# yezhen17/3DIoUMatch

Measured on AMD Instinct MI355X. Metric: scenes/sec train-step (ScanNet 40k pts, 256 proposals), higher is better.
Workload: dtype f32

## Files before the change

### 3dioumatch_amd/csrc/loss_core.h

```cpp
#pragma once
#include <math.h>

#ifndef LOSS_HD
#define LOSS_HD inline
#endif

#include "../../include/loss_hip.h"

typedef VnLossTensor LossTensor;
typedef VnLossArgs LossArgs;

LOSS_HD float lt_at(const LossTensor &t, int b, int k, int c, int d = 0) {
  return t.p[b * t.sb + k * t.sk + c * t.sc + d * t.sd];
}

enum {
  ACC_MASK, ACC_CE_MASK, ACC_POS, ACC_OBJACC, ACC_CENTER1, ACC_HCLS, ACC_HREG, ACC_SCLS, ACC_SREG,
  ACC_SEM, ACC_CLSACC, ACC_IOULAB, ACC_IOULAB_OBJ, ACC_IOUACC, ACC_IOUACC_OBJ, ACC_IOUHUB,
  ACC_JITACC, ACC_JITHUB, ACC_BLM, ACC_DIST2, ACC_VMASK, ACC_VDIST, ACC_COUNT
};

enum {
  ST_LOSS = VN_ST_LOSS, ST_VOTE = VN_ST_VOTE, ST_OBJ = VN_ST_OBJ, ST_CENTER = VN_ST_CENTER,
  ST_HCLS = VN_ST_HCLS, ST_HREG = VN_ST_HREG, ST_SCLS = VN_ST_SCLS, ST_SREG = VN_ST_SREG,
  ST_SEM = VN_ST_SEM, ST_BOX = VN_ST_BOX, ST_IOU = VN_ST_IOU, ST_JIT = VN_ST_JIT,
  ST_POS_RATIO = VN_ST_POS_RATIO, ST_NEG_RATIO = VN_ST_NEG_RATIO, ST_OBJ_ACC = VN_ST_OBJ_ACC,
  ST_OBJ_COUNT = VN_ST_OBJ_COUNT, ST_CLS_ACC = VN_ST_CLS_ACC, ST_PRED_IOU = VN_ST_PRED_IOU,
  ST_PRED_IOU_OBJ = VN_ST_PRED_IOU_OBJ, ST_IOU_ACC = VN_ST_IOU_ACC,
  ST_IOU_ACC_OBJ = VN_ST_IOU_ACC_OBJ, ST_JIT_ACC = VN_ST_JIT_ACC,
  ST_JIT_ACC_OBJ = VN_ST_JIT_ACC_OBJ, ST_COUNT = VN_ST_COUNT
};

constexpr int kLossBlock = 256;
LOSS_HD int loss_blocks_per_scene(int k, int s) {
  return (k + kLossBlock - 1) / kLossBlock + 1 + (s + kLossBlock - 1) / kLossBlock;
}

constexpr float kLossWeight = 10.0f;
constexpr float kNear = 0.3f, kFar = 0.6f;

LOSS_HD float huber1(float x) {
  const float a = fabsf(x);
  return a <= 1.0f ? 0.5f * x * x : a - 0.5f;
}
LOSS_HD float huber1_grad(float x) { return x > 1.0f ? 1.0f : (x < -1.0f ? -1.0f : x); }

constexpr int kRowMax = 32;

struct ScoreRow {
  float v[kRowMax];
};

LOSS_HD void load_row(const LossTensor &t, int b, int k, int n, ScoreRow &r) {
#pragma unroll
  for (int j = 0; j < kRowMax; ++j) r.v[j] = j < n ? lt_at(t, b, k, j) : -INFINITY;
}

LOSS_HD float row_log_sum_exp(const ScoreRow &r) {
  float m = r.v[0];
#pragma unroll
  for (int j = 1; j < kRowMax; ++j) m = r.v[j] > m ? r.v[j] : m;
  float s = 0.0f;
#pragma unroll
  for (int j = 0; j < kRowMax; ++j) s += expf(r.v[j] - m);
  return m + logf(s);
}

LOSS_HD float log_sum_exp(const LossTensor &t, int b, int k, int n) {
  float m = lt_at(t, b, k, 0);
  for (int j = 1; j < n; ++j) { const float v = lt_at(t, b, k, j); m = v > m ? v : m; }
  float s = 0.0f;
  for (int j = 0; j < n; ++j) s += expf(lt_at(t, b, k, j) - m);
  return m + logf(s);
}

LOSS_HD int arg_max(const LossTensor &t, int b, int k, int n) {
  int best = 0;
  float m = lt_at(t, b, k, 0);
  for (int j = 1; j < n; ++j) { const float v = lt_at(t, b, k, j); if (v > m) { m = v; best = j; } }
  return best;
}

LOSS_HD int row_arg_max(const LossTensor &t, int b, int k, int n) {
  if (n > kRowMax) return arg_max(t, b, k, n);
  ScoreRow r;
  load_row(t, b, k, n, r);
  int best = 0;
  float m = r.v[0];
#pragma unroll
  for (int j = 1; j < kRowMax; ++j)
    if (r.v[j] > m) { m = r.v[j]; best = j; }
  return best;
}

LOSS_HD float ce_and_grad(const LossTensor &t, int b, int k, int n, int label, float scale, float *g,
                          int *top) {
  if (n <= kRowMax) {
    ScoreRow r;
    load_row(t, b, k, n, r);
    const float lse = row_log_sum_exp(r);
    float at_label = 0.0f, m = r.v[0];
    int best = 0;
#pragma unroll
    for (int j = 0; j < kRowMax; ++j) {
      if (j < n) {
        g[j] = scale * (expf(r.v[j] - lse) - (j == label ? 1.0f : 0.0f));
        if (j == label) at_label = r.v[j];
        if (r.v[j] > m) { m = r.v[j]; best = j; }
      }
    }
    *top = best;
    return lse - at_label;
  }
  const float lse = log_sum_exp(t, b, k, n);
  for (int j = 0; j < n; ++j)
    g[j] = scale * (expf(lt_at(t, b, k, j) - lse) - (j == label ? 1.0f : 0.0f));
  *top = arg_max(t, b, k, n);
  return lse - lt_at(t, b, k, label);
}

LOSS_HD float class2angle(int cls, float residual, int nh) {
  if (nh == 1) return 0.0f;
  const float per = (float)(2.0 * M_PI / (double)nh);
  float angle = (float)cls * per + residual;
  if (angle > (float)M_PI) angle = angle - (float)(2.0 * M_PI);
  return angle;
}

LOSS_HD void decode_prediction(const LossArgs &a, int b, int k) {
  const int rows = a.has_jitter ? 2 * a.K : a.K;
  float *o = a.boxes + ((long long)b * rows + k) * 7;
  const int hc = row_arg_max(a.h_scores, b, k, a.NH);
  const int sc = row_arg_max(a.s_scores, b, k, a.NS);
  const float h_res = lt_at(a.h_resn, b, k, hc) * (float)(M_PI / (double)a.NH);
  for (int d = 0; d < 3; ++d) {
    o[d] = lt_at(a.center, b, k, d);
    const float mean = a.mean_size[sc * 3 + d];
    float s = mean + lt_at(a.s_resn, b, k, sc, d) * mean;
    if (s <= 0.0f) s = 1e-6f;
    o[3 + d] = s;
  }
  o[6] = -class2angle(hc, h_res, a.NH);
  if (a.has_jitter) {
    float *j = a.boxes + ((long long)b * rows + a.K + k) * 7;
    for (int d = 0; d < 3; ++d) {
      j[d] = lt_at(a.jit_center, b, k, d);
      j[3 + d] = lt_at(a.jit_size, b, k, d);
    }
    j[6] = -lt_at(a.jit_heading, b, k, 0);
  }
}

LOSS_HD void decode_ground_truth(const LossArgs &a, int b, int g) {
  const long long i = (long long)b * a.G + g;
  float *o = a.gt_boxes + i * 7;
  const bool empty = a.box_label_mask[i] != 1.0f;
  const int sc = (int)a.size_class_label[i];
  for (int d = 0; d < 3; ++d) {
    o[d] = empty ? -1000.0f : a.center_label[i * 3 + d];
    o[3 + d] = a.mean_size[sc * 3 + d] + a.size_residual_label[i * 3 + d];
  }
  o[6] = -class2angle((int)a.heading_class_label[i], a.heading_residual_label[i], a.NH);
}

struct SceneView {
  const float *gt_center;
  const float *gt_mask;
  const float *center;
  const int *nearest;
};

LOSS_HD void loss_proposal(const LossArgs &a, const SceneView &sv, int b, int k, float *acc) {
  const long long bk = (long long)b * a.K + k;
  const float vx = lt_at(a.agg_xyz, b, k, 0), vy = lt_at(a.agg_xyz, b, k, 1), vz = lt_at(a.agg_xyz, b, k, 2);
  const float cx = lt_at(a.center, b, k, 0), cy = lt_at(a.center, b, k, 1), cz = lt_at(a.center, b, k, 2);
  float best = 0.0f, best_c = 0.0f;
  int assign = 0, near_c = 0;
  for (int g = 0; g < a.G; ++g) {
    const float gx = sv.gt_center[g * 3], gy = sv.gt_center[g * 3 + 1], gz = sv.gt_center[g * 3 + 2];
    const bool empty = sv.gt_mask[g] != 1.0f;
    const float mx = empty ? -1000.0f : gx, my = empty ? -1000.0f : gy, mz = empty ? -1000.0f : gz;
    const float d = ((vx - mx) * (vx - mx) + (vy - my) * (vy - my)) + (vz - mz) * (vz - mz);
    if (g == 0 || d < best) { best = d; assign = g; }
    const float dc = ((cx - gx) * (cx - gx) + (cy - gy) * (cy - gy)) + (cz - gz) * (cz - gz);
    if (g == 0 || dc < best_c) { best_c = dc; near_c = g; }
  }
  const float dist = sqrtf(best + 1e-6f);
  const int label = dist < kNear ? 1 : 0;
  const float mask = (dist < kNear || dist > kFar) ? 1.0f : 0.0f;
  const float obj = (float)label;
  a.objectness_label[bk] = label;
  a.objectness_mask[bk] = mask;
  a.object_assignment[bk] = assign;
  acc[ACC_MASK] += mask;
  acc[ACC_POS] += obj;

  {
    const float w = label ? 0.8f : 0.2f;
    const float s0 = lt_at(a.obj, b, k, 0), s1 = lt_at(a.obj, b, k, 1);
    const float m = s0 > s1 ? s0 : s1;
    const float lse = m + logf(expf(s0 - m) + expf(s1 - m));
    const float scale = (a.consistency ? 0.0f : 0.5f * kLossWeight) * mask * w;
    a.g_obj[bk * 2] = scale * (expf(s0 - lse) - (label == 0 ? 1.0f : 0.0f));
    a.g_obj[bk * 2 + 1] = scale * (expf(s1 - lse) - (label == 1 ? 1.0f : 0.0f));
    acc[ACC_CE_MASK] += w * (lse - (label ? s1 : s0)) * mask;
    acc[ACC_OBJACC] += ((s1 > s0 ? 1 : 0) == label ? 1.0f : 0.0f) * mask;
  }
  {
    acc[ACC_CENTER1] += best_c * obj;
    const float s = kLossWeight * obj * 2.0f;
    a.g_center[bk * 3 + 0] = s * (cx - sv.gt_center[near_c * 3 + 0]);
    a.g_center[bk * 3 + 1] = s * (cy - sv.gt_center[near_c * 3 + 1]);
    a.g_center[bk * 3 + 2] = s * (cz - sv.gt_center[near_c * 3 + 2]);
  }
  const long long gi = (long long)b * a.G + assign;
  {
    const int hl = (int)a.heading_class_label[gi];
    float *gs = a.g_h_scores + bk * a.NH, *gr = a.g_h_resn + bk * a.NH;
    int top;
    acc[ACC_HCLS] += obj * ce_and_grad(a.h_scores, b, k, a.NH, hl, 0.1f * kLossWeight * obj, gs, &top);
    const float target = a.heading_residual_label[gi] / (float)(M_PI / (double)a.NH);
    const float x = lt_at(a.h_resn, b, k, hl) - target;
    acc[ACC_HREG] += obj * huber1(x);
    for (int j = 0; j < a.NH; ++j) gr[j] = j == hl ? kLossWeight * obj * huber1_grad(x) : 0.0f;
  }
  {
    const int sl = (int)a.size_class_label[gi];
    float *gs = a.g_s_scores + bk * a.NS, *gr = a.g_s_resn + bk * a.NS * 3;
    int top;
    acc[ACC_SCLS] += obj * ce_and_grad(a.s_scores, b, k, a.NS, sl, 0.1f * kLossWeight * obj, gs, &top);
    for (int j = 0; j < a.NS * 3; ++j) gr[j] = 0.0f;
    float reg = 0.0f;
    for (int d = 0; d < 3; ++d) {
      const float x = lt_at(a.s_resn, b, k, sl, d) - a.size_residual_label[gi * 3 + d] / a.mean_size[sl * 3 + d];
      reg += huber1(x);
      gr[sl * 3 + d] = kLossWeight * obj * huber1_grad(x) / 3.0f;
    }
    acc[ACC_SREG] += obj * (reg / 3.0f);
  }
  {
    const int cl = (int)a.sem_cls_label[gi];
    int top;
    acc[ACC_SEM] += obj * ce_and_grad(a.sem, b, k, a.NC, cl, 0.1f * kLossWeight * obj,
                                      a.g_sem + bk * a.NC, &top);
    acc[ACC_CLSACC] += obj * (top == cl ? 1.0f : 0.0f);
  }
  if (a.consistency) return;
  const int rows = a.has_jitter ? 2 * a.K : a.K;
  {
    const long long r = (long long)b * rows + k;
    const float lab = a.iou_lab[r];
    const int sel = a.NI > 1 ? (int)a.sem_cls_label[(long long)b * a.G + a.iou_assign[r]] : 0;
    const float p = 1.0f / (1.0f + expf(-lt_at(a.iou, b, k, sel)));
    const float x = p - lab;
    acc[ACC_IOULAB] += lab;
    acc[ACC_IOULAB_OBJ] += lab * obj;
    acc[ACC_IOUACC] += fabsf(x);
    acc[ACC_IOUACC_OBJ] += fabsf(x) * obj;
    acc[ACC_IOUHUB] += huber1(x);
    const float s = a.grad_scale * kLossWeight / (float)(a.B * a.K) * huber1_grad(x) * p * (1.0f - p);
    for (int j = 0; j < a.NI; ++j) a.g_iou[bk * a.NI + j] = j == sel ? s : 0.0f;
  }
  if (a.has_jitter) {
    const long long r = (long long)b * rows + a.K + k;
    const float lab = a.iou_lab[r];
    const int sel = a.NI > 1 ? (int)a.sem_cls_label[(long long)b * a.G + a.iou_assign[r]] : 0;
    const float p = 1.0f / (1.0f + expf(-lt_at(a.iou_jit, b, k, sel)));
    const float x = p - lab;
    acc[ACC_JITACC] += fabsf(x);
    acc[ACC_JITHUB] += huber1(x);
    const float s = a.grad_scale * kLossWeight / ((float)(a.B * a.K) + 1e-6f) * huber1_grad(x) * p * (1.0f - p);
    for (int j = 0; j < a.NI; ++j) a.g_iou_jit[bk * a.NI + j] = j == sel ? s : 0.0f;
  }
}

LOSS_HD void loss_ground_truth(const LossArgs &a, const SceneView &sv, int b, int g, float *acc) {
  const long long i = (long long)b * a.G + g;
  const float gx = sv.gt_center[g * 3], gy = sv.gt_center[g * 3 + 1], gz = sv.gt_center[g * 3 + 2];
  float best = 0.0f;
  int arg = 0;
  for (int k = 0; k < a.K; ++k) {
    const float cx = sv.center[k * 3], cy = sv.center[k * 3 + 1], cz = sv.center[k * 3 + 2];
    const float d = ((cx - gx) * (cx - gx) + (cy - gy) * (cy - gy)) + (cz - gz) * (cz - gz);
    if (k == 0 || d < best) { best = d; arg = k; }
  }
  a.gt_nearest[i] = arg;
  acc[ACC_BLM] += sv.gt_mask[g];
  acc[ACC_DIST2] += best * sv.gt_mask[g];
}

LOSS_HD int loss_seed(const LossArgs &a, int b, int s, float *acc, float *m) {
  const int p = a.seed_inds[b * a.seed_inds_stride + s];
  const long long row = (long long)b * a.N + p;
  const float mask = (float)a.vote_label_mask[row];
  float best = 0.0f;
  int arg = 0;
  for (int j = 0; j < a.VF; ++j)
    for (int g = 0; g < 3; ++g) {
      float d = 0.0f;
      for (int c = 0; c < 3; ++c)
        d += fabsf(lt_at(a.vote_xyz, b, s * a.VF + j, c) -
                   (a.vote_label[row * 9 + g * 3 + c] + lt_at(a.seed_xyz, b, s, c)));
      if ((j == 0 && g == 0) || d < best) { best = d; arg = j * 3 + g; }
    }
  acc[ACC_VMASK] += mask;
  acc[ACC_VDIST] += best * mask;
  *m = mask;
  return arg;
}

LOSS_HD void loss_stats(const LossArgs &a, const float *acc) {
  float *st = a.stats;
  const float total = (float)(a.B * a.K);
  const float cnt = acc[ACC_POS];
  const float inv = 1.0f / (cnt + 1e-6f);
  st[ST_VOTE] = acc[ACC_VDIST] / (acc[ACC_VMASK] + 1e-6f);
  st[ST_OBJ] = acc[ACC_CE_MASK] / (acc[ACC_MASK] + 1e-6f);
  st[ST_CENTER] = acc[ACC_CENTER1] * inv + acc[ACC_DIST2] / (acc[ACC_BLM] + 1e-6f);
  st[ST_HCLS] = acc[ACC_HCLS] * inv;
  st[ST_HREG] = acc[ACC_HREG] * inv;
  st[ST_SCLS] = acc[ACC_SCLS] * inv;
  st[ST_SREG] = acc[ACC_SREG] * inv;
  st[ST_SEM] = acc[ACC_SEM] * inv;
  st[ST_BOX] = 0.1f * st[ST_HCLS] + st[ST_HREG] + 0.1f * st[ST_SCLS] + st[ST_SREG] + st[ST_CENTER];
  st[ST_IOU] = acc[ACC_IOUHUB] / total;
  st[ST_JIT] = a.has_jitter ? acc[ACC_JITHUB] / (total + 1e-6f) : 0.0f;
  st[ST_LOSS] = kLossWeight * (st[ST_VOTE] + 0.5f * st[ST_OBJ] + st[ST_BOX] + 0.1f * st[ST_SEM] +
                               st[ST_IOU] + st[ST_JIT]);
  if (a.consistency) {
    st[ST_VOTE] = st[ST_IOU] = st[ST_JIT] = 0.0f;
    st[ST_LOSS] = kLossWeight * (st[ST_BOX] + 0.1f * st[ST_SEM]);
  }
  st[ST_POS_RATIO] = cnt / total;
  st[ST_NEG_RATIO] = acc[ACC_MASK] / total - st[ST_POS_RATIO];
  st[ST_OBJ_ACC] = acc[ACC_OBJACC] / (acc[ACC_MASK] + 1e-6f);
  st[ST_OBJ_COUNT] = cnt;
  st[ST_CLS_ACC] = acc[ACC_CLSACC] * inv;
  st[ST_PRED_IOU] = acc[ACC_IOULAB] / total;
  st[ST_PRED_IOU_OBJ] = acc[ACC_IOULAB_OBJ] * inv;
  st[ST_IOU_ACC] = acc[ACC_IOUACC] / total;
  st[ST_IOU_ACC_OBJ] = acc[ACC_IOUACC_OBJ] * inv;
  st[ST_JIT_ACC] = a.has_jitter ? acc[ACC_JITACC] / total : 0.0f;
  st[ST_JIT_ACC_OBJ] = a.has_jitter ? acc[ACC_JITACC] / (total + 1e-6f) : 0.0f;
}

LOSS_HD void finalize_proposal(const LossArgs &a, const SceneView &sv, int b, int k, const float *acc) {
  const long long bk = (long long)b * a.K + k;
  const float so = a.grad_scale / (acc[ACC_MASK] + 1e-6f), sp = a.grad_scale / (acc[ACC_POS] + 1e-6f);
  a.g_obj[bk * 2] *= so;
  a.g_obj[bk * 2 + 1] *= so;
  float back[3] = {0.0f, 0.0f, 0.0f};
  const float sb = a.grad_scale * kLossWeight / (acc[ACC_BLM] + 1e-6f) * 2.0f;
  for (int g = 0; g < a.G; ++g)
    if (sv.nearest[g] == k)
      for (int d = 0; d < 3; ++d)
        back[d] += sb * sv.gt_mask[g] * (lt_at(a.center, b, k, d) - sv.gt_center[g * 3 + d]);
  for (int d = 0; d < 3; ++d) a.g_center[bk * 3 + d] = a.g_center[bk * 3 + d] * sp + back[d];
  for (int j = 0; j < a.NH; ++j) { a.g_h_scores[bk * a.NH + j] *= sp; a.g_h_resn[bk * a.NH + j] *= sp; }
  for (int j = 0; j < a.NS; ++j) a.g_s_scores[bk * a.NS + j] *= sp;
  for (int j = 0; j < a.NS * 3; ++j) a.g_s_resn[bk * a.NS * 3 + j] *= sp;
  for (int j = 0; j < a.NC; ++j) a.g_sem[bk * a.NC + j] *= sp;
}

LOSS_HD void vote_grad(const LossArgs &a, int b, int s, int arg, float mask, const float *acc) {
  const int p = a.seed_inds[b * a.seed_inds_stride + s];
  const long long row = (long long)b * a.N + p;
  const float scale = a.grad_scale * kLossWeight * mask / (acc[ACC_VMASK] + 1e-6f);
  for (int j = 0; j < a.VF; ++j)
    for (int c = 0; c < 3; ++c) {
      float v = 0.0f;
      if (j == arg / 3) {
        const float x = lt_at(a.vote_xyz, b, s * a.VF + j, c) -
                        (a.vote_label[row * 9 + (arg % 3) * 3 + c] + lt_at(a.seed_xyz, b, s, c));
        v = scale * (x > 0.0f ? 1.0f : (x < 0.0f ? -1.0f : 0.0f));
      }
      a.g_vote[((long long)b * a.S * a.VF + s * a.VF + j) * 3 + c] = v;
    }
}

enum { EV_ACC_CLSACC_OBJ = ACC_JITACC };

enum {
  EV_LOSS = VN_EV_LOSS, EV_VOTE = VN_EV_VOTE, EV_OBJ = VN_EV_OBJ, EV_CENTER = VN_EV_CENTER,
  EV_HCLS = VN_EV_HCLS, EV_HREG = VN_EV_HREG, EV_SCLS = VN_EV_SCLS, EV_SREG = VN_EV_SREG,
  EV_SEM = VN_EV_SEM, EV_BOX = VN_EV_BOX, EV_IOU = VN_EV_IOU, EV_POS_RATIO = VN_EV_POS_RATIO,
  EV_NEG_RATIO = VN_EV_NEG_RATIO, EV_OBJ_ACC = VN_EV_OBJ_ACC, EV_CLS_ACC = VN_EV_CLS_ACC,
  EV_CLS_ACC_OBJ = VN_EV_CLS_ACC_OBJ, EV_PRED_IOU = VN_EV_PRED_IOU,
  EV_PRED_IOU_OBJ = VN_EV_PRED_IOU_OBJ, EV_IOU_ACC = VN_EV_IOU_ACC,
  EV_IOU_ACC_OBJ = VN_EV_IOU_ACC_OBJ, EV_OBJ_COUNT = VN_EV_OBJ_COUNT, EV_COUNT = VN_EV_COUNT
};

LOSS_HD float ce_forward(const LossTensor &t, int b, int k, int n, int label, int *top) {
  if (n <= kRowMax) {
    ScoreRow r;
    load_row(t, b, k, n, r);
    const float lse = row_log_sum_exp(r);
    float at_label = 0.0f, m = r.v[0];
    int best = 0;
#pragma unroll
    for (int j = 0; j < kRowMax; ++j) {
      if (j < n) {
        if (j == label) at_label = r.v[j];
        if (r.v[j] > m) { m = r.v[j]; best = j; }
      }
    }
    *top = best;
    return lse - at_label;
  }
  *top = arg_max(t, b, k, n);
  return log_sum_exp(t, b, k, n) - lt_at(t, b, k, label);
}

LOSS_HD void eval_decode_prediction(const LossArgs &a, int b, int k) {
  float *o = a.boxes + ((long long)b * a.K + k) * 7;
  const int hc = row_arg_max(a.h_scores, b, k, a.NH);
  const int sc = row_arg_max(a.s_scores, b, k, a.NS);
  const float h_res = lt_at(a.h_resn, b, k, hc) * (float)(M_PI / (double)a.NH);
  for (int d = 0; d < 3; ++d) {
    o[d] = lt_at(a.center, b, k, d);
    float s = a.mean_size[sc * 3 + d] + lt_at(a.jit_size, b, k, sc, d);
    if (s <= 0.0f) s = 1e-6f;
    o[3 + d] = s;
  }
  o[6] = -class2angle(hc, h_res, a.NH);
}

LOSS_HD void eval_proposal(const LossArgs &a, const SceneView &sv, int b, int k, float *acc) {
  const long long bk = (long long)b * a.K + k;
  const float vx = lt_at(a.agg_xyz, b, k, 0), vy = lt_at(a.agg_xyz, b, k, 1), vz = lt_at(a.agg_xyz, b, k, 2);
  const float cx = lt_at(a.center, b, k, 0), cy = lt_at(a.center, b, k, 1), cz = lt_at(a.center, b, k, 2);
  float best = 0.0f, best_c = 0.0f;
  int assign = 0;
  for (int g = 0; g < a.G; ++g) {
    const float gx = sv.gt_center[g * 3], gy = sv.gt_center[g * 3 + 1], gz = sv.gt_center[g * 3 + 2];
    const float d = ((vx - gx) * (vx - gx) + (vy - gy) * (vy - gy)) + (vz - gz) * (vz - gz);
    if (g == 0 || d < best) { best = d; assign = g; }
    const float dc = ((cx - gx) * (cx - gx) + (cy - gy) * (cy - gy)) + (cz - gz) * (cz - gz);
    if (g == 0 || dc < best_c) best_c = dc;
  }
  const float dist = sqrtf(best + 1e-6f);
  const int label = dist < kNear ? 1 : 0;
  const float mask = (dist < kNear || dist > kFar) ? 1.0f : 0.0f;
  const float obj = (float)label;
  a.objectness_label[bk] = label;
  a.objectness_mask[bk] = mask;
  a.object_assignment[bk] = assign;
  acc[ACC_MASK] += mask;
  acc[ACC_POS] += obj;
  {
    const float w = label ? 0.8f : 0.2f;
    const float s0 = lt_at(a.obj, b, k, 0), s1 = lt_at(a.obj, b, k, 1);
    const float m = s0 > s1 ? s0 : s1;
    const float lse = m + logf(expf(s0 - m) + expf(s1 - m));
    acc[ACC_CE_MASK] += w * (lse - (label ? s1 : s0)) * mask;
    acc[ACC_OBJACC] += ((s1 > s0 ? 1 : 0) == label ? 1.0f : 0.0f) * mask;
  }
  acc[ACC_CENTER1] += best_c * obj;
  const long long gi = (long long)b * a.G + assign;
  int top;
  {
    const int hl = (int)a.heading_class_label[gi];
    acc[ACC_HCLS] += obj * ce_forward(a.h_scores, b, k, a.NH, hl, &top);
    const float target = a.heading_residual_label[gi] / (float)(M_PI / (double)a.NH);
    acc[ACC_HREG] += obj * huber1(lt_at(a.h_resn, b, k, hl) - target);
  }
  {
    const int sl = (int)a.size_class_label[gi];
    acc[ACC_SCLS] += obj * ce_forward(a.s_scores, b, k, a.NS, sl, &top);
    float reg = 0.0f;
    for (int d = 0; d < 3; ++d)
      reg += huber1(lt_at(a.s_resn, b, k, sl, d) - a.size_residual_label[gi * 3 + d] / a.mean_size[sl * 3 + d]);
    acc[ACC_SREG] += obj * (reg / 3.0f);
  }
  {
    const int cl = (int)a.sem_cls_label[gi];
    acc[ACC_SEM] += obj * ce_forward(a.sem, b, k, a.NC, cl, &top);
    const float match = top == cl ? 1.0f : 0.0f;
    acc[ACC_CLSACC] += match;
    acc[EV_ACC_CLSACC_OBJ] += match * obj;
  }
  {
    const float lab = a.iou_lab[bk];
    const float p = 1.0f / (1.0f + expf(-lt_at(a.iou, b, k, a.NI > 1 ? top : 0)));
    const float x = p - lab;
    acc[ACC_IOULAB] += lab;
    acc[ACC_IOULAB_OBJ] += lab * obj;
    acc[ACC_IOUACC] += fabsf(x);
    acc[ACC_IOUACC_OBJ] += fabsf(x) * obj;
    acc[ACC_IOUHUB] += huber1(x) * obj;
  }
}

LOSS_HD void eval_ground_truth(const LossArgs &a, const SceneView &sv, int g, float *acc) {
  const float gx = sv.gt_center[g * 3], gy = sv.gt_center[g * 3 + 1], gz = sv.gt_center[g * 3 + 2];
  float best = 0.0f;
  for (int k = 0; k < a.K; ++k) {
    const float cx = sv.center[k * 3], cy = sv.center[k * 3 + 1], cz = sv.center[k * 3 + 2];
    const float d = ((cx - gx) * (cx - gx) + (cy - gy) * (cy - gy)) + (cz - gz) * (cz - gz);
    if (k == 0 || d < best) best = d;
  }
  acc[ACC_BLM] += sv.gt_mask[g];
  acc[ACC_DIST2] += best * sv.gt_mask[g];
}

LOSS_HD void eval_stats(const LossArgs &a, const float *acc, float *st, float *accum) {
  const float total = (float)(a.B * a.K);
  const float cnt = acc[ACC_POS];
  const float inv = 1.0f / (cnt + 1e-6f);
  st[EV_VOTE] = acc[ACC_VDIST] / (acc[ACC_VMASK] + 1e-6f);
  st[EV_OBJ] = acc[ACC_CE_MASK] / (acc[ACC_MASK] + 1e-6f);
  st[EV_CENTER] = acc[ACC_CENTER1] * inv + acc[ACC_DIST2] / (acc[ACC_BLM] + 1e-6f);
  st[EV_HCLS] = acc[ACC_HCLS] * inv;
  st[EV_HREG] = acc[ACC_HREG] * inv;
  st[EV_SCLS] = acc[ACC_SCLS] * inv;
  st[EV_SREG] = acc[ACC_SREG] * inv;
  st[EV_SEM] = acc[ACC_SEM] * inv;
  st[EV_BOX] = 0.1f * st[EV_HCLS] + st[EV_HREG] + 0.1f * st[EV_SCLS] + st[EV_SREG] + st[EV_CENTER];
  st[EV_IOU] = acc[ACC_IOUHUB] * inv;
  st[EV_LOSS] = kLossWeight * (st[EV_VOTE] + 0.5f * st[EV_OBJ] + st[EV_BOX] + 0.1f * st[EV_SEM] + st[EV_IOU]);
  st[EV_POS_RATIO] = cnt / total;
  st[EV_NEG_RATIO] = acc[ACC_MASK] / total - st[EV_POS_RATIO];
  st[EV_OBJ_ACC] = acc[ACC_OBJACC] / (acc[ACC_MASK] + 1e-6f);
  st[EV_CLS_ACC] = acc[ACC_CLSACC] / total;
  st[EV_CLS_ACC_OBJ] = acc[EV_ACC_CLSACC_OBJ] * inv;
  st[EV_PRED_IOU] = acc[ACC_IOULAB] / total;
  st[EV_PRED_IOU_OBJ] = acc[ACC_IOULAB_OBJ] * inv;
  st[EV_IOU_ACC] = acc[ACC_IOUACC] / total;
  st[EV_IOU_ACC_OBJ] = acc[ACC_IOUACC_OBJ] * inv;
  st[EV_OBJ_COUNT] = cnt;
  if (accum)
    for (int i = 0; i < EV_COUNT; ++i) accum[i] += st[i];
}
```

### 3dioumatch_amd/csrc/votenet_loss.hip

```cpp
#include "common.h"
#define LOSS_HD __host__ __device__ __forceinline__
#include "loss_core.h"

namespace {

constexpr int kMaxG = 256, kMaxK = 2048;

__global__ void __launch_bounds__(256) loss_decode_kernel(LossArgs a) {
  const int item = blockIdx.x * blockDim.x + threadIdx.x;
  const int props = a.B * a.K;
  if (item < props) {
    decode_prediction(a, item / a.K, item % a.K);
  } else if (item < props + a.B * a.G) {
    const int t = item - props;
    decode_ground_truth(a, t / a.G, t % a.G);
  }
}

struct Roles {
  int proposal_blocks, gt_block, per_scene;
};

__device__ __forceinline__ Roles roles(const LossArgs &a) {
  Roles r;
  r.proposal_blocks = (a.K + kLossBlock - 1) / kLossBlock;
  r.gt_block = r.proposal_blocks;
  r.per_scene = loss_blocks_per_scene(a.K, a.S);
  return r;
}

__device__ __forceinline__ void stage_ground_truth(const LossArgs &a, int b, float *gtc, float *gtm) {
  for (int t = threadIdx.x; t < a.G * 3; t += kLossBlock) gtc[t] = a.center_label[(long long)b * a.G * 3 + t];
  for (int t = threadIdx.x; t < a.G; t += kLossBlock) gtm[t] = a.box_label_mask[(long long)b * a.G + t];
}

__device__ __forceinline__ void write_partial_row(const float (&acc)[ACC_COUNT],
                                                  float (&partial)[kLossBlock / kWave][ACC_COUNT], float *row) {
  const int tid = threadIdx.x, lane = lane_id(), wave = tid / kWave;
#pragma unroll
  for (int i = 0; i < ACC_COUNT; ++i) {
    float v = acc[i];
    for (int off = kWave / 2; off > 0; off >>= 1) v += __shfl_down(v, off, kWave);
    if (lane == 0) partial[wave][i] = v;
  }
  __syncthreads();
  if (tid < ACC_COUNT) {
    float v = 0.0f;
    for (int w = 0; w < kLossBlock / kWave; ++w) v += partial[w][tid];
    row[tid] = v;
  }
}

__device__ __forceinline__ void sum_partial_rows(const LossArgs &a, int rows, float (&share)[kLossBlock / 32][32],
                                                 float *total) {
  const int tid = threadIdx.x, col = tid & 31, group = tid >> 5;
  float v = 0.0f;
  if (col < ACC_COUNT)
    for (int row = group; row < rows; row += kLossBlock / 32)
      v += a.partials[(long long)row * ACC_COUNT + col];
  share[group][col] = v;
  __syncthreads();
  if (tid < ACC_COUNT) {
    float t = 0.0f;
    for (int g = 0; g < kLossBlock / 32; ++g) t += share[g][tid];
    total[tid] = t;
  }
}

__global__ void __launch_bounds__(kLossBlock) loss_terms_kernel(LossArgs a) {
  __shared__ float gtc[kMaxG * 3], gtm[kMaxG], ctr[kMaxK * 3];
  __shared__ float partial[kLossBlock / kWave][ACC_COUNT];
  const Roles r = roles(a);
  const int role = blockIdx.x, b = blockIdx.y, tid = threadIdx.x;
  stage_ground_truth(a, b, gtc, gtm);
  if (role == r.gt_block)
    for (int t = tid; t < a.K * 3; t += kLossBlock) ctr[t] = lt_at(a.center, b, t / 3, t % 3);
  __syncthreads();
  SceneView sv;
  sv.gt_center = gtc; sv.gt_mask = gtm; sv.center = ctr; sv.nearest = nullptr;
  float acc[ACC_COUNT];
#pragma unroll
  for (int i = 0; i < ACC_COUNT; ++i) acc[i] = 0.0f;
  if (role < r.proposal_blocks) {
    const int k = role * kLossBlock + tid;
    if (k < a.K) loss_proposal(a, sv, b, k, acc);
  } else if (role == r.gt_block) {
    for (int g = tid; g < a.G; g += kLossBlock) loss_ground_truth(a, sv, b, g, acc);
  } else {
    const int s = (role - r.gt_block - 1) * kLossBlock + tid;
    float m;
    if (s < a.S) loss_seed(a, b, s, acc, &m);
  }
  write_partial_row(acc, partial, a.partials + ((long long)b * r.per_scene + role) * ACC_COUNT);
}

__global__ void __launch_bounds__(kLossBlock) loss_finalize_kernel(LossArgs a) {
  __shared__ float gtc[kMaxG * 3], gtm[kMaxG];
  __shared__ int nearest[kMaxG];
  __shared__ float total[ACC_COUNT];
  __shared__ float share[kLossBlock / 32][32];
  const Roles r = roles(a);
  const int role = blockIdx.x, b = blockIdx.y, tid = threadIdx.x;
  sum_partial_rows(a, a.B * r.per_scene, share, total);
  if (role < r.proposal_blocks) {
    stage_ground_truth(a, b, gtc, gtm);
    for (int t = tid; t < a.G; t += kLossBlock) nearest[t] = a.gt_nearest[(long long)b * a.G + t];
  }
  __syncthreads();
  float acc[ACC_COUNT];
#pragma unroll
  for (int i = 0; i < ACC_COUNT; ++i) acc[i] = total[i];
  if (role < r.proposal_blocks) {
    SceneView sv;
    sv.gt_center = gtc; sv.gt_mask = gtm; sv.center = nullptr; sv.nearest = nearest;
    const int k = role * kLossBlock + tid;
    if (k < a.K) finalize_proposal(a, sv, b, k, acc);
  } else if (role == r.gt_block) {
    if (b == 0 && tid == 0) loss_stats(a, acc);
  } else {
    const int s = (role - r.gt_block - 1) * kLossBlock + tid;
    if (s < a.S) {
      float scratch[ACC_COUNT] = {}, m;
      const int arg = loss_seed(a, b, s, scratch, &m);
      vote_grad(a, b, s, arg, m, acc);
    }
  }
}

__global__ void __launch_bounds__(256) eval_decode_kernel(LossArgs a) {
  const int item = blockIdx.x * blockDim.x + threadIdx.x;
  const int props = a.B * a.K;
  if (item < props) {
    eval_decode_prediction(a, item / a.K, item % a.K);
  } else if (item < props + a.B * a.G) {
    const int t = item - props;
    decode_ground_truth(a, t / a.G, t % a.G);
  }
}

__global__ void __launch_bounds__(kLossBlock) eval_terms_kernel(LossArgs a) {
  __shared__ float gtc[kMaxG * 3], gtm[kMaxG], ctr[kMaxK * 3];
  __shared__ float partial[kLossBlock / kWave][ACC_COUNT];
  const Roles r = roles(a);
  const int role = blockIdx.x, b = blockIdx.y, tid = threadIdx.x;
  stage_ground_truth(a, b, gtc, gtm);
  if (role == r.gt_block)
    for (int t = tid; t < a.K * 3; t += kLossBlock) ctr[t] = lt_at(a.center, b, t / 3, t % 3);
  __syncthreads();
  SceneView sv;
  sv.gt_center = gtc; sv.gt_mask = gtm; sv.center = ctr; sv.nearest = nullptr;
  float acc[ACC_COUNT];
#pragma unroll
  for (int i = 0; i < ACC_COUNT; ++i) acc[i] = 0.0f;
  if (role < r.proposal_blocks) {
    const int k = role * kLossBlock + tid;
    if (k < a.K) eval_proposal(a, sv, b, k, acc);
  } else if (role == r.gt_block) {
    for (int g = tid; g < a.G; g += kLossBlock) eval_ground_truth(a, sv, g, acc);
  } else {
    const int s = (role - r.gt_block - 1) * kLossBlock + tid;
    float m;
    if (s < a.S) loss_seed(a, b, s, acc, &m);
  }
  write_partial_row(acc, partial, a.partials + ((long long)b * r.per_scene + role) * ACC_COUNT);
}

__global__ void __launch_bounds__(kLossBlock) eval_stats_kernel(LossArgs a, float *stats, float *accum) {
  __shared__ float total[ACC_COUNT];
  __shared__ float share[kLossBlock / 32][32];
  sum_partial_rows(a, a.B * roles(a).per_scene, share, total);
  __syncthreads();
  if (threadIdx.x == 0) eval_stats(a, total, stats, accum);
}

bool valid(const VnLossArgs *a) {
  if (a && a->consistency && (a->S != 0 || a->VF != 0)) return false;
  return a && a->B > 0 && a->K > 0 && a->G > 0 && (a->consistency || (a->S > 0 && a->VF > 0)) && a->NH > 0 && a->NS > 0 &&
         a->NC > 0 && (a->NI == 1 || a->NI == a->NC) && a->G <= kMaxG && a->K <= kMaxK &&
         a->B <= 65535;
}

}

extern "C" __attribute__((visibility("default")))
int votenet_loss_scratch_floats(const VnLossArgs *args) {
  if (!valid(args)) return 0;
  return args->B * loss_blocks_per_scene(args->K, args->S) * ACC_COUNT;
}

extern "C" __attribute__((visibility("default")))
int votenet_loss_decode(const VnLossArgs *args, void *stream) {
  if (!valid(args)) return (int)hipErrorInvalidValue;
  const int items = args->B * (args->K + args->G);
  hipLaunchKernelGGL(loss_decode_kernel, dim3((items + 255) / 256), dim3(256), 0,
                     (hipStream_t)stream, *args);
  return (int)hipGetLastError();
}

extern "C" __attribute__((visibility("default")))
int votenet_loss_forward_backward(const VnLossArgs *args, void *stream) {
  if (!valid(args) || !args->partials) return (int)hipErrorInvalidValue;
  const dim3 grid(loss_blocks_per_scene(args->K, args->S), args->B);
  hipLaunchKernelGGL(loss_terms_kernel, grid, dim3(kLossBlock), 0, (hipStream_t)stream, *args);
  hipLaunchKernelGGL(loss_finalize_kernel, grid, dim3(kLossBlock), 0, (hipStream_t)stream, *args);
  return (int)hipGetLastError();
}

namespace {
bool eval_valid(const VnLossArgs *a) {
  if (!a) return false;
  VnLossArgs plain = *a;
  plain.consistency = 0;
  return valid(&plain);
}
}

extern "C" __attribute__((visibility("default")))
int votenet_eval_loss_decode(const VnLossArgs *args, void *stream) {
  if (!eval_valid(args)) return (int)hipErrorInvalidValue;
  const int items = args->B * (args->K + args->G);
  hipLaunchKernelGGL(eval_decode_kernel, dim3((items + 255) / 256), dim3(256), 0, (hipStream_t)stream, *args);
  return (int)hipGetLastError();
}

extern "C" __attribute__((visibility("default")))
int votenet_eval_loss(const VnLossArgs *args, float *stats, float *accum, void *stream) {
  if (!eval_valid(args) || !args->partials || !stats) return (int)hipErrorInvalidValue;
  const dim3 grid(loss_blocks_per_scene(args->K, args->S), args->B);
  hipLaunchKernelGGL(eval_terms_kernel, grid, dim3(kLossBlock), 0, (hipStream_t)stream, *args);
  hipLaunchKernelGGL(eval_stats_kernel, dim3(1), dim3(kLossBlock), 0, (hipStream_t)stream, *args, stats, accum);
  return (int)hipGetLastError();
}


namespace {

struct DecodeArgs {
  int b, k, nh, ns, nc;
  const float *net, *agg_xyz, *mean_size;
  float *objectness, *center, *heading_scores, *heading_resn, *heading_res, *size_scores, *size_resn,
      *size_res, *sem_cls;
};

__device__ __forceinline__ float softplus1(float x) {
  return x > 20.0f ? x : log1pf(expf(x));
}

__global__ void __launch_bounds__(256) decode_scores_kernel(DecodeArgs a) {
  const int c_total = 5 + 2 * a.nh + 4 * a.ns + a.nc;
  const long long t = (long long)blockIdx.x * 256 + threadIdx.x;
  if (t >= (long long)a.b * c_total * a.k) return;
  const int ki = (int)(t % a.k);
  const long long bc = t / a.k;
  const int c = (int)(bc % c_total), bi = (int)(bc / c_total);
  const long long i = (long long)bi * a.k + ki;
  const float v = a.net[t];
  int j = c;
  if (j < 2) { a.objectness[i * 2 + j] = v; return; }
  j -= 2;
  if (j < 3) { a.center[i * 3 + j] = a.agg_xyz[i * 3 + j] + v; return; }
  j -= 3;
  if (j < a.nh) { a.heading_scores[i * a.nh + j] = v; return; }
  j -= a.nh;
  if (j < a.nh) {
    const float per = (float)(M_PI / (double)a.nh);
    a.heading_resn[i * a.nh + j] = v;
    a.heading_res[i * a.nh + j] = v * per;
    return;
  }
  j -= a.nh;
  if (j < a.ns) { a.size_scores[i * a.ns + j] = v; return; }
  j -= a.ns;
  if (j < a.ns * 3) {
    const float u = softplus1(v) - 1.0f;
    a.size_resn[i * a.ns * 3 + j] = u;
    a.size_res[i * a.ns * 3 + j] = u * a.mean_size[j];
    return;
  }
  j -= a.ns * 3;
  a.sem_cls[i * a.nc + j] = v;
}

struct DecodeGradArgs {
  int b, k, nh, ns, nc;
  const float *net, *mean_size;
  const float *g_objectness, *g_center, *g_heading_scores, *g_heading_resn, *g_heading_res,
      *g_size_scores, *g_size_resn, *g_size_res, *g_sem_cls;
  float *d_net;
};

__global__ void __launch_bounds__(256) decode_scores_grad_kernel(DecodeGradArgs a) {
  const int c_total = 5 + 2 * a.nh + 4 * a.ns + a.nc;
  const long long t = (long long)blockIdx.x * 256 + threadIdx.x;
  if (t >= (long long)a.b * c_total * a.k) return;
  const int ki = (int)(t % a.k);
  const long long bc = t / a.k;
  const int c = (int)(bc % c_total), bi = (int)(bc / c_total);
  const long long i = (long long)bi * a.k + ki;
  auto get = [&](const float *g, long long at) { return g ? g[at] : 0.0f; };
  int j = c;
  float out;
  if (j < 2) {
    out = get(a.g_objectness, i * 2 + j);
  } else if ((j -= 2) < 3) {
    out = get(a.g_center, i * 3 + j);
  } else if ((j -= 3) < a.nh) {
    out = get(a.g_heading_scores, i * a.nh + j);
  } else if ((j -= a.nh) < a.nh) {
    const float per = (float)(M_PI / (double)a.nh);
    out = get(a.g_heading_resn, i * a.nh + j) + get(a.g_heading_res, i * a.nh + j) * per;
  } else if ((j -= a.nh) < a.ns) {
    out = get(a.g_size_scores, i * a.ns + j);
  } else if ((j -= a.ns) < a.ns * 3) {
    const float x = a.net[t];
    const float slope = x > 20.0f ? 1.0f : 1.0f / (1.0f + expf(-x));
    const float g = get(a.g_size_resn, i * a.ns * 3 + j) + get(a.g_size_res, i * a.ns * 3 + j) * a.mean_size[j];
    out = g * slope;
  } else {
    j -= a.ns * 3;
    out = get(a.g_sem_cls, i * a.nc + j);
  }
  a.d_net[t] = out;
}

}

extern "C" __attribute__((visibility("default")))
int votenet_decode_scores(int b, int k, int nh, int ns, int nc, const float *net, const float *agg_xyz,
                          const float *mean_size, float *objectness, float *center,
                          float *heading_scores, float *heading_resn, float *heading_res,
                          float *size_scores, float *size_resn, float *size_res, float *sem_cls,
                          void *stream) {
  if (b <= 0 || k <= 0) return 0;
  if (nh <= 0 || ns <= 0 || nc <= 0) return (int)hipErrorInvalidValue;
  const DecodeArgs a = {b, k, nh, ns, nc, net, agg_xyz, mean_size, objectness, center, heading_scores,
                        heading_resn, heading_res, size_scores, size_resn, size_res, sem_cls};
  const long long total = (long long)b * (5 + 2 * nh + 4 * ns + nc) * k;
  hipLaunchKernelGGL(decode_scores_kernel, dim3((unsigned)((total + 255) / 256)), dim3(256), 0,
                     (hipStream_t)stream, a);
  return (int)hipGetLastError();
}

extern "C" __attribute__((visibility("default")))
int votenet_decode_scores_grad(int b, int k, int nh, int ns, int nc, const float *net,
                               const float *mean_size, const float *g_objectness, const float *g_center,
                               const float *g_heading_scores, const float *g_heading_resn,
                               const float *g_heading_res, const float *g_size_scores,
                               const float *g_size_resn, const float *g_size_res, const float *g_sem_cls,
                               float *d_net, void *stream) {
  if (b <= 0 || k <= 0) return 0;
  if (nh <= 0 || ns <= 0 || nc <= 0) return (int)hipErrorInvalidValue;
  const DecodeGradArgs a = {b, k, nh, ns, nc, net, mean_size, g_objectness, g_center, g_heading_scores,
                            g_heading_resn, g_heading_res, g_size_scores, g_size_resn, g_size_res,
                            g_sem_cls, d_net};
  const long long total = (long long)b * (5 + 2 * nh + 4 * ns + nc) * k;
  hipLaunchKernelGGL(decode_scores_grad_kernel, dim3((unsigned)((total + 255) / 256)), dim3(256),
                     0, (hipStream_t)stream, a);
  return (int)hipGetLastError();
}

namespace {
__global__ void __launch_bounds__(256)
iou_score_slices_grad_kernel(int c_out, int kt, int iou_size, int k0, const float *__restrict__ g0,
                             const float *__restrict__ g1, float *__restrict__ d_net, long long total) {
  const long long i = (long long)blockIdx.x * 256 + threadIdx.x;
  if (i >= total) return;
  const int j = (int)(i % kt);
  const long long row = i / kt;
  const int ch = (int)(row % c_out), b = (int)(row / c_out);
  const int s = ch - (c_out - iou_size);
  float v = 0.f;
  if (s >= 0) {
    if (j < k0) v = g0 ? g0[((size_t)b * k0 + j) * iou_size + s] : 0.f;
    else v = g1 ? g1[((size_t)b * (kt - k0) + (j - k0)) * iou_size + s] : 0.f;
  }
  d_net[i] = v;
}
}

extern "C" __attribute__((visibility("default")))
int votenet_iou_score_slices_grad(int b, int c_out, int kt, int iou_size, int k0, const float *g0,
                                  const float *g1, float *d_net, void *stream_) {
  if (b <= 0 || c_out <= 0 || kt <= 0) return 0;
  if (iou_size < 0 || iou_size > c_out || k0 < 0 || k0 > kt || !d_net) return (int)hipErrorInvalidValue;
  const long long total = (long long)b * c_out * kt;
  hipLaunchKernelGGL(iou_score_slices_grad_kernel, dim3((unsigned)((total + 255) / 256)), dim3(256), 0,
                     (hipStream_t)stream_, c_out, kt, iou_size, k0, g0, g1, d_net, total);
  return (int)hipGetLastError();
}
```

Measured before the change: 1417.

## Split per-proposal loss work across lane groups and cache forward state in scratch

Restructures the training loss kernels so each proposal is handled by a group of lanes instead of a single thread, with class-row gradients, center back-terms (via wave ballot) and residual gradients written cooperatively. The forward kernel now stores per-proposal and per-seed intermediates (nearest-GT indices, log-sum-exps, seed argmin and mask) in scratch, so the gradient kernel no longer recomputes loss_seed or full distance scans. Vote gradients are written element-wise with a small unrolled lookahead for coalesced stores. In exchange it adds scratch memory traffic and more blocks per scene, and requires a larger scratch allocation.

```diff
diff --git a/3dioumatch_amd/csrc/loss_core.h b/3dioumatch_amd/csrc/loss_core.h
--- a/3dioumatch_amd/csrc/loss_core.h
+++ b/3dioumatch_amd/csrc/loss_core.h
@@ -44,6 +44,8 @@
   return a <= 1.0f ? 0.5f * x * x : a - 0.5f;
 }
 LOSS_HD float huber1_grad(float x) { return x > 1.0f ? 1.0f : (x < -1.0f ? -1.0f : x); }
+
+LOSS_HD float pick3(int d, float x0, float x1, float x2) { return d == 0 ? x0 : (d == 1 ? x1 : x2); }
 
 constexpr int kRowMax = 32;
 
@@ -91,6 +93,10 @@
   for (int j = 1; j < kRowMax; ++j)
     if (r.v[j] > m) { m = r.v[j]; best = j; }
   return best;
+}
+
+LOSS_HD float ce_grad_element(float v, float lse, bool at_label, float scale) {
+  return scale * (expf(v - lse) - (at_label ? 1.0f : 0.0f));
 }
 
 LOSS_HD float ce_and_grad(const LossTensor &t, int b, int k, int n, int label, float scale, float *g,
@@ -104,7 +110,7 @@
 #pragma unroll
     for (int j = 0; j < kRowMax; ++j) {
       if (j < n) {
-        g[j] = scale * (expf(r.v[j] - lse) - (j == label ? 1.0f : 0.0f));
+        g[j] = ce_grad_element(r.v[j], lse, j == label, scale);
         if (j == label) at_label = r.v[j];
         if (r.v[j] > m) { m = r.v[j]; best = j; }
       }
@@ -113,8 +119,7 @@
     return lse - at_label;
   }
   const float lse = log_sum_exp(t, b, k, n);
-  for (int j = 0; j < n; ++j)
-    g[j] = scale * (expf(lt_at(t, b, k, j) - lse) - (j == label ? 1.0f : 0.0f));
+  for (int j = 0; j < n; ++j) g[j] = ce_grad_element(lt_at(t, b, k, j), lse, j == label, scale);
   *top = arg_max(t, b, k, n);
   return lse - lt_at(t, b, k, label);
 }
@@ -127,27 +132,32 @@
   return angle;
 }
 
+LOSS_HD float prediction_box_element(const LossArgs &a, int b, int k, int hc, int sc, int e) {
+  if (e < 3) return lt_at(a.center, b, k, e);
+  if (e < 6) {
+    const float mean = a.mean_size[sc * 3 + (e - 3)];
+    const float s = mean + lt_at(a.s_resn, b, k, sc, e - 3) * mean;
+    return s <= 0.0f ? 1e-6f : s;
+  }
+  const float h_res = lt_at(a.h_resn, b, k, hc) * (float)(M_PI / (double)a.NH);
+  return -class2angle(hc, h_res, a.NH);
+}
+
+LOSS_HD float jitter_box_element(const LossArgs &a, int b, int k, int e) {
+  if (e < 3) return lt_at(a.jit_center, b, k, e);
+  if (e < 6) return lt_at(a.jit_size, b, k, e - 3);
+  return -lt_at(a.jit_heading, b, k, 0);
+}
+
 LOSS_HD void decode_prediction(const LossArgs &a, int b, int k) {
   const int rows = a.has_jitter ? 2 * a.K : a.K;
   float *o = a.boxes + ((long long)b * rows + k) * 7;
   const int hc = row_arg_max(a.h_scores, b, k, a.NH);
   const int sc = row_arg_max(a.s_scores, b, k, a.NS);
-  const float h_res = lt_at(a.h_resn, b, k, hc) * (float)(M_PI / (double)a.NH);
-  for (int d = 0; d < 3; ++d) {
-    o[d] = lt_at(a.center, b, k, d);
-    const float mean = a.mean_size[sc * 3 + d];
-    float s = mean + lt_at(a.s_resn, b, k, sc, d) * mean;
-    if (s <= 0.0f) s = 1e-6f;
-    o[3 + d] = s;
-  }
-  o[6] = -class2angle(hc, h_res, a.NH);
+  for (int e = 0; e < 7; ++e) o[e] = prediction_box_element(a, b, k, hc, sc, e);
   if (a.has_jitter) {
     float *j = a.boxes + ((long long)b * rows + a.K + k) * 7;
-    for (int d = 0; d < 3; ++d) {
-      j[d] = lt_at(a.jit_center, b, k, d);
-      j[3 + d] = lt_at(a.jit_size, b, k, d);
-    }
-    j[6] = -lt_at(a.jit_heading, b, k, 0);
+    for (int e = 0; e < 7; ++e) j[e] = jitter_box_element(a, b, k, e);
   }
 }
 
@@ -170,107 +180,184 @@
   const int *nearest;
 };
 
+
+LOSS_HD bool nearer(float d, int i, float than_d, int than_i) {
+  return d < than_d || (!(than_d < d) && i < than_i);
+}
+
+LOSS_HD float center_distance2(const float *c, float gx, float gy, float gz) {
+  return ((c[0] - gx) * (c[0] - gx) + (c[1] - gy) * (c[1] - gy)) + (c[2] - gz) * (c[2] - gz);
+}
+
+LOSS_HD void gt_distances(const SceneView &sv, int g, const float *v, const float *c, float *d, float *dc) {
+  const float gx = sv.gt_center[g * 3], gy = sv.gt_center[g * 3 + 1], gz = sv.gt_center[g * 3 + 2];
+  const bool empty = sv.gt_mask[g] != 1.0f;
+  const float mx = empty ? -1000.0f : gx, my = empty ? -1000.0f : gy, mz = empty ? -1000.0f : gz;
+  *d = ((v[0] - mx) * (v[0] - mx) + (v[1] - my) * (v[1] - my)) + (v[2] - mz) * (v[2] - mz);
+  *dc = center_distance2(c, gx, gy, gz);
+}
+
+struct ProposalLabels {
+  int label, assign, near_c;
+  float mask, obj;
+  int hl, sl, cl;
+  float hx, sx[3];
+};
+
+LOSS_HD ProposalLabels proposal_labels(const LossArgs &a, int b, int k, float best, int assign, int near_c) {
+  ProposalLabels p;
+  const float dist = sqrtf(best + 1e-6f);
+  p.label = dist < kNear ? 1 : 0;
+  p.mask = (dist < kNear || dist > kFar) ? 1.0f : 0.0f;
+  p.obj = (float)p.label;
+  p.assign = assign;
+  p.near_c = near_c;
+  const long long gi = (long long)b * a.G + assign;
+  p.hl = (int)a.heading_class_label[gi];
+  p.sl = (int)a.size_class_label[gi];
+  p.cl = (int)a.sem_cls_label[gi];
+  const float target = a.heading_residual_label[gi] / (float)(M_PI / (double)a.NH);
+  p.hx = lt_at(a.h_resn, b, k, p.hl) - target;
+  for (int d = 0; d < 3; ++d)
+    p.sx[d] = lt_at(a.s_resn, b, k, p.sl, d) - a.size_residual_label[gi * 3 + d] / a.mean_size[p.sl * 3 + d];
+  return p;
+}
+
+LOSS_HD void objectness_term(const LossArgs &a, int b, int k, const ProposalLabels &p, float *acc, float *g) {
+  const float w = p.label ? 0.8f : 0.2f;
+  const float s0 = lt_at(a.obj, b, k, 0), s1 = lt_at(a.obj, b, k, 1);
+  const float m = s0 > s1 ? s0 : s1;
+  const float lse = m + logf(expf(s0 - m) + expf(s1 - m));
+  const float scale = (a.consistency ? 0.0f : 0.5f * kLossWeight) * p.mask * w;
+  g[0] = scale * (expf(s0 - lse) - (p.label == 0 ? 1.0f : 0.0f));
+  g[1] = scale * (expf(s1 - lse) - (p.label == 1 ? 1.0f : 0.0f));
+  acc[ACC_CE_MASK] += w * (lse - (p.label ? s1 : s0)) * p.mask;
+  acc[ACC_OBJACC] += ((s1 > s0 ? 1 : 0) == p.label ? 1.0f : 0.0f) * p.mask;
+}
+
+LOSS_HD float class_grad_scale(const ProposalLabels &p) { return 0.1f * kLossWeight * p.obj; }
+
+LOSS_HD float center_grad_element(const SceneView &sv, const ProposalLabels &p, float c, int d) {
+  const float s = kLossWeight * p.obj * 2.0f;
+  return s * (c - sv.gt_center[p.near_c * 3 + d]);
+}
+
+LOSS_HD float h_resn_grad_element(const ProposalLabels &p, int j) {
+  return j == p.hl ? kLossWeight * p.obj * huber1_grad(p.hx) : 0.0f;
+}
+
+LOSS_HD float s_resn_grad_element(const ProposalLabels &p, int j) {
+  const float x = pick3(j % 3, p.sx[0], p.sx[1], p.sx[2]);
+  return j / 3 == p.sl ? kLossWeight * p.obj * huber1_grad(x) / 3.0f : 0.0f;
+}
+
+LOSS_HD void box_terms(const ProposalLabels &p, float ce_h, float ce_s, float ce_sem, int top_sem, float *acc) {
+  acc[ACC_HCLS] += p.obj * ce_h;
+  acc[ACC_HREG] += p.obj * huber1(p.hx);
+  acc[ACC_SCLS] += p.obj * ce_s;
+  float reg = 0.0f;
+  for (int d = 0; d < 3; ++d) reg += huber1(p.sx[d]);
+  acc[ACC_SREG] += p.obj * (reg / 3.0f);
+  acc[ACC_SEM] += p.obj * ce_sem;
+  acc[ACC_CLSACC] += p.obj * (top_sem == p.cl ? 1.0f : 0.0f);
+}
+
+struct IouTerm {
+  int sel;
+  float lab, p, x;
+};
+
+LOSS_HD IouTerm iou_term(const LossArgs &a, const LossTensor &scores, int b, int k, long long r) {
+  IouTerm t;
+  t.lab = a.iou_lab[r];
+  t.sel = a.NI > 1 ? (int)a.sem_cls_label[(long long)b * a.G + a.iou_assign[r]] : 0;
+  t.p = 1.0f / (1.0f + expf(-lt_at(scores, b, k, t.sel)));
+  t.x = t.p - t.lab;
+  return t;
+}
+
+LOSS_HD void iou_sums(const IouTerm &t, float obj, float *acc) {
+  acc[ACC_IOULAB] += t.lab;
+  acc[ACC_IOULAB_OBJ] += t.lab * obj;
+  acc[ACC_IOUACC] += fabsf(t.x);
+  acc[ACC_IOUACC_OBJ] += fabsf(t.x) * obj;
+  acc[ACC_IOUHUB] += huber1(t.x);
+}
+
+LOSS_HD void jitter_sums(const IouTerm &t, float *acc) {
+  acc[ACC_JITACC] += fabsf(t.x);
+  acc[ACC_JITHUB] += huber1(t.x);
+}
+
+LOSS_HD float iou_grad(const LossArgs &a, const IouTerm &t, float count) {
+  return a.grad_scale * kLossWeight / count * huber1_grad(t.x) * t.p * (1.0f - t.p);
+}
+
+struct GradScales {
+  float so, sp, sb;
+};
+
+LOSS_HD GradScales grad_scales(const LossArgs &a, const float *acc) {
+  GradScales s;
+  s.so = a.grad_scale / (acc[ACC_MASK] + 1e-6f);
+  s.sp = a.grad_scale / (acc[ACC_POS] + 1e-6f);
+  s.sb = a.grad_scale * kLossWeight / (acc[ACC_BLM] + 1e-6f) * 2.0f;
+  return s;
+}
+
+LOSS_HD float center_back_term(const SceneView &sv, int g, float c, int d, float sb) {
+  return sb * sv.gt_mask[g] * (c - sv.gt_center[g * 3 + d]);
+}
+
+LOSS_HD float center_back_element(const SceneView &sv, int groups, int k, float c, int d, float sb) {
+  float back = 0.0f;
+  for (int g = 0; g < groups; ++g)
+    if (sv.nearest[g] == k) back += center_back_term(sv, g, c, d, sb);
+  return back;
+}
+
 LOSS_HD void loss_proposal(const LossArgs &a, const SceneView &sv, int b, int k, float *acc) {
   const long long bk = (long long)b * a.K + k;
-  const float vx = lt_at(a.agg_xyz, b, k, 0), vy = lt_at(a.agg_xyz, b, k, 1), vz = lt_at(a.agg_xyz, b, k, 2);
-  const float cx = lt_at(a.center, b, k, 0), cy = lt_at(a.center, b, k, 1), cz = lt_at(a.center, b, k, 2);
+  const float v[3] = {lt_at(a.agg_xyz, b, k, 0), lt_at(a.agg_xyz, b, k, 1), lt_at(a.agg_xyz, b, k, 2)};
+  const float c[3] = {lt_at(a.center, b, k, 0), lt_at(a.center, b, k, 1), lt_at(a.center, b, k, 2)};
   float best = 0.0f, best_c = 0.0f;
   int assign = 0, near_c = 0;
   for (int g = 0; g < a.G; ++g) {
-    const float gx = sv.gt_center[g * 3], gy = sv.gt_center[g * 3 + 1], gz = sv.gt_center[g * 3 + 2];
-    const bool empty = sv.gt_mask[g] != 1.0f;
-    const float mx = empty ? -1000.0f : gx, my = empty ? -1000.0f : gy, mz = empty ? -1000.0f : gz;
-    const float d = ((vx - mx) * (vx - mx) + (vy - my) * (vy - my)) + (vz - mz) * (vz - mz);
+    float d, dc;
+    gt_distances(sv, g, v, c, &d, &dc);
     if (g == 0 || d < best) { best = d; assign = g; }
-    const float dc = ((cx - gx) * (cx - gx) + (cy - gy) * (cy - gy)) + (cz - gz) * (cz - gz);
     if (g == 0 || dc < best_c) { best_c = dc; near_c = g; }
   }
-  const float dist = sqrtf(best + 1e-6f);
-  const int label = dist < kNear ? 1 : 0;
-  const float mask = (dist < kNear || dist > kFar) ? 1.0f : 0.0f;
-  const float obj = (float)label;
-  a.objectness_label[bk] = label;
-  a.objectness_mask[bk] = mask;
+  const ProposalLabels p = proposal_labels(a, b, k, best, assign, near_c);
+  a.objectness_label[bk] = p.label;
+  a.objectness_mask[bk] = p.mask;
   a.object_assignment[bk] = assign;
-  acc[ACC_MASK] += mask;
-  acc[ACC_POS] += obj;
-
-  {
-    const float w = label ? 0.8f : 0.2f;
-    const float s0 = lt_at(a.obj, b, k, 0), s1 = lt_at(a.obj, b, k, 1);
-    const float m = s0 > s1 ? s0 : s1;
-    const float lse = m + logf(expf(s0 - m) + expf(s1 - m));
-    const float scale = (a.consistency ? 0.0f : 0.5f * kLossWeight) * mask * w;
-    a.g_obj[bk * 2] = scale * (expf(s0 - lse) - (label == 0 ? 1.0f : 0.0f));
-    a.g_obj[bk * 2 + 1] = scale * (expf(s1 - lse) - (label == 1 ? 1.0f : 0.0f));
-    acc[ACC_CE_MASK] += w * (lse - (label ? s1 : s0)) * mask;
-    acc[ACC_OBJACC] += ((s1 > s0 ? 1 : 0) == label ? 1.0f : 0.0f) * mask;
-  }
-  {
-    acc[ACC_CENTER1] += best_c * obj;
-    const float s = kLossWeight * obj * 2.0f;
-    a.g_center[bk * 3 + 0] = s * (cx - sv.gt_center[near_c * 3 + 0]);
-    a.g_center[bk * 3 + 1] = s * (cy - sv.gt_center[near_c * 3 + 1]);
-    a.g_center[bk * 3 + 2] = s * (cz - sv.gt_center[near_c * 3 + 2]);
-  }
-  const long long gi = (long long)b * a.G + assign;
-  {
-    const int hl = (int)a.heading_class_label[gi];
-    float *gs = a.g_h_scores + bk * a.NH, *gr = a.g_h_resn + bk * a.NH;
-    int top;
-    acc[ACC_HCLS] += obj * ce_and_grad(a.h_scores, b, k, a.NH, hl, 0.1f * kLossWeight * obj, gs, &top);
-    const float target = a.heading_residual_label[gi] / (float)(M_PI / (double)a.NH);
-    const float x = lt_at(a.h_resn, b, k, hl) - target;
-    acc[ACC_HREG] += obj * huber1(x);
-    for (int j = 0; j < a.NH; ++j) gr[j] = j == hl ? kLossWeight * obj * huber1_grad(x) : 0.0f;
-  }
-  {
-    const int sl = (int)a.size_class_label[gi];
-    float *gs = a.g_s_scores + bk * a.NS, *gr = a.g_s_resn + bk * a.NS * 3;
-    int top;
-    acc[ACC_SCLS] += obj * ce_and_grad(a.s_scores, b, k, a.NS, sl, 0.1f * kLossWeight * obj, gs, &top);
-    for (int j = 0; j < a.NS * 3; ++j) gr[j] = 0.0f;
-    float reg = 0.0f;
-    for (int d = 0; d < 3; ++d) {
-      const float x = lt_at(a.s_resn, b, k, sl, d) - a.size_residual_label[gi * 3 + d] / a.mean_size[sl * 3 + d];
-      reg += huber1(x);
-      gr[sl * 3 + d] = kLossWeight * obj * huber1_grad(x) / 3.0f;
-    }
-    acc[ACC_SREG] += obj * (reg / 3.0f);
-  }
-  {
-    const int cl = (int)a.sem_cls_label[gi];
-    int top;
-    acc[ACC_SEM] += obj * ce_and_grad(a.sem, b, k, a.NC, cl, 0.1f * kLossWeight * obj,
-                                      a.g_sem + bk * a.NC, &top);
-    acc[ACC_CLSACC] += obj * (top == cl ? 1.0f : 0.0f);
-  }
+  acc[ACC_MASK] += p.mask;
+  acc[ACC_POS] += p.obj;
+  objectness_term(a, b, k, p, acc, a.g_obj + bk * 2);
+  acc[ACC_CENTER1] += best_c * p.obj;
+  for (int d = 0; d < 3; ++d) a.g_center[bk * 3 + d] = center_grad_element(sv, p, c[d], d);
+  int top;
+  const float scale = class_grad_scale(p);
+  const float ce_h = ce_and_grad(a.h_scores, b, k, a.NH, p.hl, scale, a.g_h_scores + bk * a.NH, &top);
+  for (int j = 0; j < a.NH; ++j) a.g_h_resn[bk * a.NH + j] = h_resn_grad_element(p, j);
+  const float ce_s = ce_and_grad(a.s_scores, b, k, a.NS, p.sl, scale, a.g_s_scores + bk * a.NS, &top);
+  for (int j = 0; j < a.NS * 3; ++j) a.g_s_resn[bk * a.NS * 3 + j] = s_resn_grad_element(p, j);
+  const float ce_sem = ce_and_grad(a.sem, b, k, a.NC, p.cl, scale, a.g_sem + bk * a.NC, &top);
+  box_terms(p, ce_h, ce_s, ce_sem, top, acc);
   if (a.consistency) return;
   const int rows = a.has_jitter ? 2 * a.K : a.K;
   {
-    const long long r = (long long)b * rows + k;
-    const float lab = a.iou_lab[r];
-    const int sel = a.NI > 1 ? (int)a.sem_cls_label[(long long)b * a.G + a.iou_assign[r]] : 0;
-    const float p = 1.0f / (1.0f + expf(-lt_at(a.iou, b, k, sel)));
-    const float x = p - lab;
-    acc[ACC_IOULAB] += lab;
-    acc[ACC_IOULAB_OBJ] += lab * obj;
-    acc[ACC_IOUACC] += fabsf(x);
-    acc[ACC_IOUACC_OBJ] += fabsf(x) * obj;
-    acc[ACC_IOUHUB] += huber1(x);
-    const float s = a.grad_scale * kLossWeight / (float)(a.B * a.K) * huber1_grad(x) * p * (1.0f - p);
-    for (int j = 0; j < a.NI; ++j) a.g_iou[bk * a.NI + j] = j == sel ? s : 0.0f;
+    const IouTerm t = iou_term(a, a.iou, b, k, (long long)b * rows + k);
+    iou_sums(t, p.obj, acc);
+    const float s = iou_grad(a, t, (float)(a.B * a.K));
+    for (int j = 0; j < a.NI; ++j) a.g_iou[bk * a.NI + j] = j == t.sel ? s : 0.0f;
   }
   if (a.has_jitter) {
-    const long long r = (long long)b * rows + a.K + k;
-    const float lab = a.iou_lab[r];
-    const int sel = a.NI > 1 ? (int)a.sem_cls_label[(long long)b * a.G + a.iou_assign[r]] : 0;
-    const float p = 1.0f / (1.0f + expf(-lt_at(a.iou_jit, b, k, sel)));
-    const float x = p - lab;
-    acc[ACC_JITACC] += fabsf(x);
-    acc[ACC_JITHUB] += huber1(x);
-    const float s = a.grad_scale * kLossWeight / ((float)(a.B * a.K) + 1e-6f) * huber1_grad(x) * p * (1.0f - p);
-    for (int j = 0; j < a.NI; ++j) a.g_iou_jit[bk * a.NI + j] = j == sel ? s : 0.0f;
+    const IouTerm t = iou_term(a, a.iou_jit, b, k, (long long)b * rows + a.K + k);
+    jitter_sums(t, acc);
+    const float s = iou_grad(a, t, (float)(a.B * a.K) + 1e-6f);
+    for (int j = 0; j < a.NI; ++j) a.g_iou_jit[bk * a.NI + j] = j == t.sel ? s : 0.0f;
   }
 }
 
@@ -280,8 +367,7 @@
   float best = 0.0f;
   int arg = 0;
   for (int k = 0; k < a.K; ++k) {
-    const float cx = sv.center[k * 3], cy = sv.center[k * 3 + 1], cz = sv.center[k * 3 + 2];
-    const float d = ((cx - gx) * (cx - gx) + (cy - gy) * (cy - gy)) + (cz - gz) * (cz - gz);
+    const float d = center_distance2(sv.center + k * 3, gx, gy, gz);
     if (k == 0 || d < best) { best = d; arg = k; }
   }
   a.gt_nearest[i] = arg;
@@ -346,36 +432,34 @@
 
 LOSS_HD void finalize_proposal(const LossArgs &a, const SceneView &sv, int b, int k, const float *acc) {
   const long long bk = (long long)b * a.K + k;
-  const float so = a.grad_scale / (acc[ACC_MASK] + 1e-6f), sp = a.grad_scale / (acc[ACC_POS] + 1e-6f);
+  const GradScales n = grad_scales(a, acc);
+  const float so = n.so, sp = n.sp;
   a.g_obj[bk * 2] *= so;
   a.g_obj[bk * 2 + 1] *= so;
-  float back[3] = {0.0f, 0.0f, 0.0f};
-  const float sb = a.grad_scale * kLossWeight / (acc[ACC_BLM] + 1e-6f) * 2.0f;
-  for (int g = 0; g < a.G; ++g)
-    if (sv.nearest[g] == k)
-      for (int d = 0; d < 3; ++d)
-        back[d] += sb * sv.gt_mask[g] * (lt_at(a.center, b, k, d) - sv.gt_center[g * 3 + d]);
-  for (int d = 0; d < 3; ++d) a.g_center[bk * 3 + d] = a.g_center[bk * 3 + d] * sp + back[d];
+  for (int d = 0; d < 3; ++d)
+    a.g_center[bk * 3 + d] = a.g_center[bk * 3 + d] * sp +
+                             center_back_element(sv, a.G, k, lt_at(a.center, b, k, d), d, n.sb);
   for (int j = 0; j < a.NH; ++j) { a.g_h_scores[bk * a.NH + j] *= sp; a.g_h_resn[bk * a.NH + j] *= sp; }
   for (int j = 0; j < a.NS; ++j) a.g_s_scores[bk * a.NS + j] *= sp;
   for (int j = 0; j < a.NS * 3; ++j) a.g_s_resn[bk * a.NS * 3 + j] *= sp;
   for (int j = 0; j < a.NC; ++j) a.g_sem[bk * a.NC + j] *= sp;
 }
 
-LOSS_HD void vote_grad(const LossArgs &a, int b, int s, int arg, float mask, const float *acc) {
+LOSS_HD float vote_grad_element(const LossArgs &a, int b, int s, int j, int c, int arg, float mask,
+                                const float *acc) {
+  if (j != arg / 3) return 0.0f;
   const int p = a.seed_inds[b * a.seed_inds_stride + s];
   const long long row = (long long)b * a.N + p;
   const float scale = a.grad_scale * kLossWeight * mask / (acc[ACC_VMASK] + 1e-6f);
+  const float x = lt_at(a.vote_xyz, b, s * a.VF + j, c) -
+                  (a.vote_label[row * 9 + (arg % 3) * 3 + c] + lt_at(a.seed_xyz, b, s, c));
+  return scale * (x > 0.0f ? 1.0f : (x < 0.0f ? -1.0f : 0.0f));
+}
+
+LOSS_HD void vote_grad(const LossArgs &a, int b, int s, int arg, float mask, const float *acc) {
   for (int j = 0; j < a.VF; ++j)
-    for (int c = 0; c < 3; ++c) {
-      float v = 0.0f;
-      if (j == arg / 3) {
-        const float x = lt_at(a.vote_xyz, b, s * a.VF + j, c) -
-                        (a.vote_label[row * 9 + (arg % 3) * 3 + c] + lt_at(a.seed_xyz, b, s, c));
-        v = scale * (x > 0.0f ? 1.0f : (x < 0.0f ? -1.0f : 0.0f));
-      }
-      a.g_vote[((long long)b * a.S * a.VF + s * a.VF + j) * 3 + c] = v;
-    }
+    for (int c = 0; c < 3; ++c)
+      a.g_vote[((long long)b * a.S * a.VF + s * a.VF + j) * 3 + c] = vote_grad_element(a, b, s, j, c, arg, mask, acc);
 }
 
 enum { EV_ACC_CLSACC_OBJ = ACC_JITACC };
diff --git a/3dioumatch_amd/csrc/votenet_loss.hip b/3dioumatch_amd/csrc/votenet_loss.hip
--- a/3dioumatch_amd/csrc/votenet_loss.hip
+++ b/3dioumatch_amd/csrc/votenet_loss.hip
@@ -6,16 +6,86 @@
 
 constexpr int kMaxG = 256, kMaxK = 2048;
 
+constexpr int kGroup = 16;
+constexpr int kGroupsPerBlock = kLossBlock / kGroup;
+constexpr int kSlotLanes = 4;
+constexpr int kNoIndex = 0x7fffffff;
+static_assert(kRowMax == 2 * kGroup, "a lane keeps elements l and l + kGroup of a row in registers");
+
+template <int W>
+__device__ __forceinline__ float group_sum(float v) {
+#pragma unroll
+  for (int off = W / 2; off >= 1; off >>= 1) v += __shfl_xor(v, off, W);
+  return v;
+}
+
+template <int W>
+__device__ __forceinline__ void group_nearest(float &d, int &i) {
+#pragma unroll
+  for (int off = W / 2; off >= 1; off >>= 1) {
+    const float od = __shfl_xor(d, off, W);
+    const int oi = __shfl_xor(i, off, W);
+    if (nearer(od, oi, d, i)) { d = od; i = oi; }
+  }
+}
+
+struct RowShare {
+  float v0, v1, max;
+  int top;
+};
+
+__device__ __forceinline__ RowShare group_row_load(const LossTensor &t, int b, int k, int n, int l) {
+  RowShare r;
+  r.v0 = l < n ? lt_at(t, b, k, l) : -INFINITY;
+  r.v1 = l + kGroup < n ? lt_at(t, b, k, l + kGroup) : -INFINITY;
+  r.max = 0.0f;
+  r.top = 0;
+  return r;
+}
+
+__device__ __forceinline__ RowShare group_row_max(RowShare r, const LossTensor &t, int b, int k, int n, int l) {
+  float neg = -r.v0;
+  int top = l < n ? l : kNoIndex;
+  if (r.v1 > r.v0) { neg = -r.v1; top = l + kGroup; }
+  for (int j = l + 2 * kGroup; j < n; j += kGroup) {
+    const float v = lt_at(t, b, k, j);
+    if (v > -neg) { neg = -v; top = j; }
+  }
+  group_nearest<kGroup>(neg, top);
+  r.max = -neg;
+  r.top = top < n ? top : 0;
+  return r;
+}
+
+__device__ __forceinline__ RowShare group_row_lse(RowShare r, const LossTensor &t, int b, int k, int n, int l) {
+  r = group_row_max(r, t, b, k, n, l);
+  float s = expf(r.v0 - r.max) + expf(r.v1 - r.max);
+  for (int j = l + 2 * kGroup; j < n; j += kGroup) s += expf(lt_at(t, b, k, j) - r.max);
+  r.max = r.max + logf(group_sum<kGroup>(s));
+  return r;
+}
+
 __global__ void __launch_bounds__(256) loss_decode_kernel(LossArgs a) {
-  const int item = blockIdx.x * blockDim.x + threadIdx.x;
-  const int props = a.B * a.K;
-  if (item < props) {
-    decode_prediction(a, item / a.K, item % a.K);
-  } else if (item < props + a.B * a.G) {
-    const int t = item - props;
-    decode_ground_truth(a, t / a.G, t % a.G);
-  }
-}
+  const long long item = (long long)blockIdx.x * 256 + threadIdx.x;
+  const long long lanes = (long long)a.B * a.K * kGroup;
+  if (item < lanes) {
+    const int l = (int)(item % kGroup);
+    const long long bk = item / kGroup;
+    const int b = (int)(bk / a.K), k = (int)(bk % a.K);
+    const RowShare h = group_row_load(a.h_scores, b, k, a.NH, l), s = group_row_load(a.s_scores, b, k, a.NS, l);
+    const int hc = group_row_max(h, a.h_scores, b, k, a.NH, l).top;
+    const int sc = group_row_max(s, a.s_scores, b, k, a.NS, l).top;
+    const long long rows = a.has_jitter ? 2 * a.K : a.K;
+    if (l < 7)
+      a.boxes[((long long)b * rows + k) * 7 + l] = prediction_box_element(a, b, k, hc, sc, l);
+    else if (l < 14 && a.has_jitter)
+      a.boxes[((long long)b * rows + a.K + k) * 7 + (l - 7)] = jitter_box_element(a, b, k, l - 7);
+  } else if (item < lanes + (long long)a.B * a.G) {
+    const long long t = item - lanes;
+    decode_ground_truth(a, (int)(t / a.G), (int)(t % a.G));
+  }
+}
+
 
 struct Roles {
   int proposal_blocks, gt_block, per_scene;
@@ -54,24 +124,172 @@
 __device__ __forceinline__ void sum_partial_rows(const LossArgs &a, int rows, float (&share)[kLossBlock / 32][32],
                                                  float *total) {
   const int tid = threadIdx.x, col = tid & 31, group = tid >> 5;
+  constexpr int kGroups = kLossBlock / 32, kAhead = 8;
   float v = 0.0f;
   if (col < ACC_COUNT)
-    for (int row = group; row < rows; row += kLossBlock / 32)
-      v += a.partials[(long long)row * ACC_COUNT + col];
+    for (int row = group; row < rows; row += kGroups * kAhead) {
+      float x[kAhead];
+#pragma unroll
+      for (int u = 0; u < kAhead; ++u) {
+        const int at = row + u * kGroups;
+        x[u] = at < rows ? a.partials[(long long)at * ACC_COUNT + col] : 0.0f;
+      }
+#pragma unroll
+      for (int u = 0; u < kAhead; ++u) v += x[u];
+    }
   share[group][col] = v;
   __syncthreads();
   if (tid < ACC_COUNT) {
     float t = 0.0f;
-    for (int g = 0; g < kLossBlock / 32; ++g) t += share[g][tid];
+    for (int g = 0; g < kGroups; ++g) t += share[g][tid];
     total[tid] = t;
   }
+}
+
+__device__ __forceinline__ void sum_count_columns(const LossArgs &a, int rows, float (&share)[kLossBlock / 32][32],
+                                                  float *total) {
+  const int tid = threadIdx.x, c = tid & 3, group = tid >> 2;
+  const int col = c == 0 ? ACC_MASK : (c == 1 ? ACC_POS : (c == 2 ? ACC_BLM : ACC_VMASK));
+  constexpr int kGroups = kLossBlock / 4, kAhead = 4;
+  float v = 0.0f;
+  for (int row = group; row < rows; row += kGroups * kAhead) {
+    float x[kAhead];
+#pragma unroll
+    for (int u = 0; u < kAhead; ++u) {
+      const int at = row + u * kGroups;
+      x[u] = at < rows ? a.partials[(long long)at * ACC_COUNT + col] : 0.0f;
+    }
+#pragma unroll
+    for (int u = 0; u < kAhead; ++u) v += x[u];
+  }
+  v += __shfl_xor(v, 4, kWave);
+  v += __shfl_xor(v, 8, kWave);
+  v += __shfl_xor(v, 16, kWave);
+  v += __shfl_xor(v, 32, kWave);
+  if (lane_id() < 4) share[tid / kWave][c] = v;
+  __syncthreads();
+  if (tid < 4) total[col] = (share[0][c] + share[1][c]) + (share[2][c] + share[3][c]);
+}
+
+__host__ __device__ __forceinline__ int train_proposal_blocks(int k) { return (k + kGroupsPerBlock - 1) / kGroupsPerBlock; }
+__host__ __device__ __forceinline__ int train_blocks_per_scene(int k, int s) {
+  return train_proposal_blocks(k) + 1 + (s + kLossBlock - 1) / kLossBlock;
+}
+
+__device__ __forceinline__ Roles train_roles(const LossArgs &a) {
+  Roles r;
+  r.proposal_blocks = train_proposal_blocks(a.K);
+  r.gt_block = r.proposal_blocks;
+  r.per_scene = train_blocks_per_scene(a.K, a.S);
+  return r;
+}
+
+enum { PS_ASSIGN, PS_NEAR_C, PS_BEST, PS_LSE_H, PS_LSE_S, PS_LSE_SEM, PS_COUNT };
+enum { SS_ARG, SS_MASK, SS_COUNT };
+
+__host__ __device__ __forceinline__ long long train_scratch_floats(const LossArgs &a) {
+  return (long long)a.B * train_blocks_per_scene(a.K, a.S) * ACC_COUNT + (long long)a.B * a.K * PS_COUNT +
+         (long long)a.B * a.S * SS_COUNT;
+}
+__device__ __forceinline__ float *proposal_scratch(const LossArgs &a, long long bk) {
+  return a.partials + (long long)a.B * train_blocks_per_scene(a.K, a.S) * ACC_COUNT + bk * PS_COUNT;
+}
+__device__ __forceinline__ float *seed_scratch(const LossArgs &a, long long bs) {
+  return proposal_scratch(a, (long long)a.B * a.K) + bs * SS_COUNT;
+}
+
+struct ProposalInputs {
+  float v[3], c[3];
+  RowShare h, s, m;
+  IouTerm iou, jit;
+};
+
+__device__ __forceinline__ ProposalInputs load_proposal(const LossArgs &a, int b, int k, int l) {
+  ProposalInputs in;
+  for (int d = 0; d < 3; ++d) { in.v[d] = lt_at(a.agg_xyz, b, k, d); in.c[d] = lt_at(a.center, b, k, d); }
+  in.h = group_row_load(a.h_scores, b, k, a.NH, l);
+  in.s = group_row_load(a.s_scores, b, k, a.NS, l);
+  in.m = group_row_load(a.sem, b, k, a.NC, l);
+  in.iou = in.jit = IouTerm();
+  if (!a.consistency) {
+    const long long rows = a.has_jitter ? 2 * a.K : a.K;
+    in.iou = iou_term(a, a.iou, b, k, b * rows + k);
+    if (a.has_jitter) in.jit = iou_term(a, a.iou_jit, b, k, b * rows + a.K + k);
+  }
+  return in;
+}
+
+__device__ __forceinline__ void terms_proposal(const LossArgs &a, const SceneView &sv, const ProposalInputs &in,
+                                               int b, int k, int l, float (&acc)[ACC_COUNT]) {
+  const long long bk = (long long)b * a.K + k;
+  float best = INFINITY, best_c = INFINITY;
+  int assign = kNoIndex, near_c = kNoIndex;
+  for (int g = l; g < a.G; g += kGroup) {
+    float d, dc;
+    gt_distances(sv, g, in.v, in.c, &d, &dc);
+    if (assign == kNoIndex || d < best) { best = d; assign = g; }
+    if (near_c == kNoIndex || dc < best_c) { best_c = dc; near_c = g; }
+  }
+  group_nearest<kGroup>(best, assign);
+  group_nearest<kGroup>(best_c, near_c);
+  const ProposalLabels p = proposal_labels(a, b, k, best, assign, near_c);
+  float sum[ACC_COUNT];
+#pragma unroll
+  for (int i = 0; i < ACC_COUNT; ++i) sum[i] = 0.0f;
+  sum[ACC_MASK] += p.mask;
+  sum[ACC_POS] += p.obj;
+  float g_obj[2];
+  objectness_term(a, b, k, p, sum, g_obj);
+  sum[ACC_CENTER1] += best_c * p.obj;
+  const float at_h = lt_at(a.h_scores, b, k, p.hl), at_s = lt_at(a.s_scores, b, k, p.sl), at_m = lt_at(a.sem, b, k, p.cl);
+  const RowShare h = group_row_lse(in.h, a.h_scores, b, k, a.NH, l);
+  const RowShare s = group_row_lse(in.s, a.s_scores, b, k, a.NS, l);
+  const RowShare m = group_row_lse(in.m, a.sem, b, k, a.NC, l);
+  box_terms(p, h.max - at_h, s.max - at_s, m.max - at_m, m.top, sum);
+  if (!a.consistency) {
+    iou_sums(in.iou, p.obj, sum);
+    if (a.has_jitter) jitter_sums(in.jit, sum);
+  }
+  if (l != 0) return;
+  a.objectness_label[bk] = p.label;
+  a.objectness_mask[bk] = p.mask;
+  a.object_assignment[bk] = assign;
+  float *keep = proposal_scratch(a, bk);
+  keep[PS_ASSIGN] = __int_as_float(assign);
+  keep[PS_NEAR_C] = __int_as_float(near_c);
+  keep[PS_BEST] = best;
+  keep[PS_LSE_H] = h.max;
+  keep[PS_LSE_S] = s.max;
+  keep[PS_LSE_SEM] = m.max;
+#pragma unroll
+  for (int i = 0; i < ACC_COUNT; ++i) acc[i] += sum[i];
+}
+
+__device__ __forceinline__ void terms_ground_truth(const LossArgs &a, const SceneView &sv, int b, int g, int l,
+                                                   float (&acc)[ACC_COUNT]) {
+  const float *at = sv.gt_center + g * 3;
+  float best = INFINITY;
+  int arg = kNoIndex;
+  for (int k = l; k < a.K; k += kSlotLanes) {
+    const float d = center_distance2(sv.center + k * 3, at[0], at[1], at[2]);
+    if (arg == kNoIndex || d < best) { best = d; arg = k; }
+  }
+  group_nearest<kSlotLanes>(best, arg);
+  if (l != 0) return;
+  a.gt_nearest[(long long)b * a.G + g] = arg;
+  acc[ACC_BLM] += sv.gt_mask[g];
+  acc[ACC_DIST2] += best * sv.gt_mask[g];
 }
 
 __global__ void __launch_bounds__(kLossBlock) loss_terms_kernel(LossArgs a) {
   __shared__ float gtc[kMaxG * 3], gtm[kMaxG], ctr[kMaxK * 3];
   __shared__ float partial[kLossBlock / kWave][ACC_COUNT];
-  const Roles r = roles(a);
+  const Roles r = train_roles(a);
   const int role = blockIdx.x, b = blockIdx.y, tid = threadIdx.x;
+  const int k = role * kGroupsPerBlock + tid / kGroup;
+  const bool proposal = role < r.proposal_blocks && k < a.K;
+  ProposalInputs in;
+  if (proposal) in = load_proposal(a, b, k, tid % kGroup);
   stage_ground_truth(a, b, gtc, gtm);
   if (role == r.gt_block)
     for (int t = tid; t < a.K * 3; t += kLossBlock) ctr[t] = lt_at(a.center, b, t / 3, t % 3);
@@ -82,50 +300,132 @@
 #pragma unroll
   for (int i = 0; i < ACC_COUNT; ++i) acc[i] = 0.0f;
   if (role < r.proposal_blocks) {
-    const int k = role * kLossBlock + tid;
-    if (k < a.K) loss_proposal(a, sv, b, k, acc);
+    if (proposal) terms_proposal(a, sv, in, b, k, tid % kGroup, acc);
   } else if (role == r.gt_block) {
-    for (int g = tid; g < a.G; g += kLossBlock) loss_ground_truth(a, sv, b, g, acc);
+    for (int first = 0; first < a.G; first += kLossBlock / kSlotLanes) {
+      const int g = first + tid / kSlotLanes;
+      if (g < a.G) terms_ground_truth(a, sv, b, g, tid % kSlotLanes, acc);
+    }
   } else {
     const int s = (role - r.gt_block - 1) * kLossBlock + tid;
-    float m;
-    if (s < a.S) loss_seed(a, b, s, acc, &m);
+    if (s < a.S) {
+      float *keep = seed_scratch(a, (long long)b * a.S + s);
+      keep[SS_ARG] = __int_as_float(loss_seed(a, b, s, acc, &keep[SS_MASK]));
+    }
   }
   write_partial_row(acc, partial, a.partials + ((long long)b * r.per_scene + role) * ACC_COUNT);
 }
 
-__global__ void __launch_bounds__(kLossBlock) loss_finalize_kernel(LossArgs a) {
+struct GradInputs {
+  ProposalInputs in;
+  ProposalLabels p;
+  float lse_h, lse_s, lse_m, g_obj0, g_obj1;
+};
+
+__device__ __forceinline__ GradInputs load_grad_inputs(const LossArgs &a, int b, int k, int l) {
+  GradInputs g;
+  const float *keep = proposal_scratch(a, (long long)b * a.K + k);
+  const float best = keep[PS_BEST];
+  const int assign = __float_as_int(keep[PS_ASSIGN]), near_c = __float_as_int(keep[PS_NEAR_C]);
+  g.lse_h = keep[PS_LSE_H];
+  g.lse_s = keep[PS_LSE_S];
+  g.lse_m = keep[PS_LSE_SEM];
+  g.in = load_proposal(a, b, k, l);
+  g.p = proposal_labels(a, b, k, best, assign, near_c);
+  float unused[ACC_COUNT], g_obj[2];
+#pragma unroll
+  for (int i = 0; i < ACC_COUNT; ++i) unused[i] = 0.0f;
+  objectness_term(a, b, k, g.p, unused, g_obj);
+  g.g_obj0 = g_obj[0];
+  g.g_obj1 = g_obj[1];
+  return g;
+}
+
+__device__ __forceinline__ void store_class_row(float *g, const LossTensor &t, const RowShare &r, int b, int k, int n,
+                                                int l, float lse, int label, float scale, float sp) {
+  if (l < n) g[l] = ce_grad_element(r.v0, lse, l == label, scale) * sp;
+  if (l + kGroup < n) g[l + kGroup] = ce_grad_element(r.v1, lse, l + kGroup == label, scale) * sp;
+  for (int j = l + 2 * kGroup; j < n; j += kGroup) g[j] = ce_grad_element(lt_at(t, b, k, j), lse, j == label, scale) * sp;
+}
+
+__device__ __forceinline__ void grad_proposal(const LossArgs &a, const SceneView &sv, const GradInputs &in, int b,
+                                              int k, int l, const float *total) {
+  const long long bk = (long long)b * a.K + k;
+  const ProposalLabels &p = in.p;
+  const GradScales n = grad_scales(a, total);
+  const int d = l < 3 ? l : 0, first_lane = lane_id() & ~(kGroup - 1);
+  const float c = pick3(d, in.in.c[0], in.in.c[1], in.in.c[2]);
+  float back = 0.0f;
+  for (int first = 0; first < a.G; first += kGroup) {
+    const int g = first + l;
+    const unsigned long long wave = __ballot(g < a.G && sv.nearest[g] == k);
+    for (unsigned hits = (unsigned)(wave >> first_lane) & ((1u << kGroup) - 1u); hits; hits &= hits - 1)
+      back += center_back_term(sv, first + __builtin_ctz(hits), c, d, n.sb);
+  }
+  if (l < 2) a.g_obj[bk * 2 + l] = pick3(l, in.g_obj0, in.g_obj1, 0.0f) * n.so;
+  if (l < 3) a.g_center[bk * 3 + l] = center_grad_element(sv, p, c, l) * n.sp + back;
+  const float scale = class_grad_scale(p);
+  store_class_row(a.g_h_scores + bk * a.NH, a.h_scores, in.in.h, b, k, a.NH, l, in.lse_h, p.hl, scale, n.sp);
+  for (int j = l; j < a.NH; j += kGroup) a.g_h_resn[bk * a.NH + j] = h_resn_grad_element(p, j) * n.sp;
+  store_class_row(a.g_s_scores + bk * a.NS, a.s_scores, in.in.s, b, k, a.NS, l, in.lse_s, p.sl, scale, n.sp);
+  for (int j = l; j < a.NS * 3; j += kGroup) a.g_s_resn[bk * a.NS * 3 + j] = s_resn_grad_element(p, j) * n.sp;
+  store_class_row(a.g_sem + bk * a.NC, a.sem, in.in.m, b, k, a.NC, l, in.lse_m, p.cl, scale, n.sp);
+  if (a.consistency) return;
+  const float si = iou_grad(a, in.in.iou, (float)(a.B * a.K));
+  for (int j = l; j < a.NI; j += kGroup) a.g_iou[bk * a.NI + j] = j == in.in.iou.sel ? si : 0.0f;
+  if (a.has_jitter) {
+    const float sj = iou_grad(a, in.in.jit, (float)(a.B * a.K) + 1e-6f);
+    for (int j = l; j < a.NI; j += kGroup) a.g_iou_jit[bk * a.NI + j] = j == in.in.jit.sel ? sj : 0.0f;
+  }
+}
+
+__global__ void __launch_bounds__(kLossBlock) loss_grad_kernel(LossArgs a) {
   __shared__ float gtc[kMaxG * 3], gtm[kMaxG];
   __shared__ int nearest[kMaxG];
   __shared__ float total[ACC_COUNT];
   __shared__ float share[kLossBlock / 32][32];
-  const Roles r = roles(a);
+  const Roles r = train_roles(a);
   const int role = blockIdx.x, b = blockIdx.y, tid = threadIdx.x;
-  sum_partial_rows(a, a.B * r.per_scene, share, total);
+  const int k = role * kGroupsPerBlock + tid / kGroup;
   if (role < r.proposal_blocks) {
+    const GradInputs in = load_grad_inputs(a, b, k < a.K ? k : a.K - 1, tid % kGroup);
     stage_ground_truth(a, b, gtc, gtm);
     for (int t = tid; t < a.G; t += kLossBlock) nearest[t] = a.gt_nearest[(long long)b * a.G + t];
-  }
-  __syncthreads();
-  float acc[ACC_COUNT];
-#pragma unroll
-  for (int i = 0; i < ACC_COUNT; ++i) acc[i] = total[i];
-  if (role < r.proposal_blocks) {
+    sum_count_columns(a, a.B * r.per_scene, share, total);
+    __syncthreads();
     SceneView sv;
     sv.gt_center = gtc; sv.gt_mask = gtm; sv.center = nullptr; sv.nearest = nearest;
-    const int k = role * kLossBlock + tid;
-    if (k < a.K) finalize_proposal(a, sv, b, k, acc);
+    if (k < a.K) grad_proposal(a, sv, in, b, k, tid % kGroup, total);
   } else if (role == r.gt_block) {
-    if (b == 0 && tid == 0) loss_stats(a, acc);
+    if (b != 0) return;
+    sum_partial_rows(a, a.B * r.per_scene, share, total);
+    __syncthreads();
+    if (tid == 0) loss_stats(a, total);
   } else {
-    const int s = (role - r.gt_block - 1) * kLossBlock + tid;
-    if (s < a.S) {
-      float scratch[ACC_COUNT] = {}, m;
-      const int arg = loss_seed(a, b, s, scratch, &m);
-      vote_grad(a, b, s, arg, m, acc);
+    sum_count_columns(a, a.B * r.per_scene, share, total);
+    __syncthreads();
+    const int first = (role - r.gt_block - 1) * kLossBlock, per = a.VF * 3;
+    constexpr int kAhead = 4;
+    for (int e0 = tid; e0 < kLossBlock * per; e0 += kLossBlock * kAhead) {
+      float v[kAhead];
+#pragma unroll
+      for (int u = 0; u < kAhead; ++u) {
+        const int e = e0 + u * kLossBlock, s = first + e / per;
+        v[u] = 0.0f;
+        if (e < kLossBlock * per && s < a.S) {
+          const float *keep = seed_scratch(a, (long long)b * a.S + s);
+          v[u] = vote_grad_element(a, b, s, (e / 3) % a.VF, e % 3, __float_as_int(keep[SS_ARG]), keep[SS_MASK], total);
+        }
+      }
+#pragma unroll
+      for (int u = 0; u < kAhead; ++u) {
+        const int e = e0 + u * kLossBlock;
+        if (e < kLossBlock * per && first + e / per < a.S) a.g_vote[((long long)b * a.S + first) * per + e] = v[u];
+      }
     }
   }
 }
+
 
 __global__ void __launch_bounds__(256) eval_decode_kernel(LossArgs a) {
   const int item = blockIdx.x * blockDim.x + threadIdx.x;
@@ -185,14 +485,15 @@
 extern "C" __attribute__((visibility("default")))
 int votenet_loss_scratch_floats(const VnLossArgs *args) {
   if (!valid(args)) return 0;
-  return args->B * loss_blocks_per_scene(args->K, args->S) * ACC_COUNT;
+  const long long floats = train_scratch_floats(*args);
+  return floats <= 0x7fffffffLL ? (int)floats : 0;
 }
 
 extern "C" __attribute__((visibility("default")))
 int votenet_loss_decode(const VnLossArgs *args, void *stream) {
   if (!valid(args)) return (int)hipErrorInvalidValue;
-  const int items = args->B * (args->K + args->G);
-  hipLaunchKernelGGL(loss_decode_kernel, dim3((items + 255) / 256), dim3(256), 0,
+  const long long items = (long long)args->B * ((long long)args->K * kGroup + args->G);
+  hipLaunchKernelGGL(loss_decode_kernel, dim3((unsigned)((items + 255) / 256)), dim3(256), 0,
                      (hipStream_t)stream, *args);
   return (int)hipGetLastError();
 }
@@ -200,9 +501,10 @@
 extern "C" __attribute__((visibility("default")))
 int votenet_loss_forward_backward(const VnLossArgs *args, void *stream) {
   if (!valid(args) || !args->partials) return (int)hipErrorInvalidValue;
-  const dim3 grid(loss_blocks_per_scene(args->K, args->S), args->B);
+  if (votenet_loss_scratch_floats(args) == 0) return (int)hipErrorInvalidValue;
+  const dim3 grid(train_blocks_per_scene(args->K, args->S), args->B);
   hipLaunchKernelGGL(loss_terms_kernel, grid, dim3(kLossBlock), 0, (hipStream_t)stream, *args);
-  hipLaunchKernelGGL(loss_finalize_kernel, grid, dim3(kLossBlock), 0, (hipStream_t)stream, *args);
+  hipLaunchKernelGGL(loss_grad_kernel, grid, dim3(kLossBlock), 0, (hipStream_t)stream, *args);
   return (int)hipGetLastError();
 }
 
```

Result: no change. 1410 (-0.5%).
